# nico-bohlinger/RL-X

Hardware: NVIDIA H100
Metric: env-steps/sec (PPO update incl.) (higher is better)
Workload: dtype f32

## Files before the change

### include/rlx_b200.h

```cpp
#ifndef RLX_B200_H
#define RLX_B200_H

#include <stddef.h>
#include <stdint.h>

#ifdef __cplusplus
extern "C" {
#endif

#define RLX_OK 0
#define RLX_ERR_INVALID_ARG (-1)
#define RLX_ERR_CUDA (-2)
#define RLX_ERR_WORKSPACE (-3)
#define RLX_ERR_UNSUPPORTED (-4)

int rlx_version(void);
const char* rlx_last_error_string(void);
uint64_t rlx_launch_count(void);
void rlx_reset_launch_count(void);
void rlx_add_launch_count(uint64_t n);
#define RLX_NKCLASS 14
int rlx_timing_begin(void);
int rlx_timing_end(double* ms, uint64_t* launches, double* flops, double* bytes);
const char* rlx_kernel_class_name(int cls);
int rlx_set_gemm_engine(int engine);
int rlx_get_gemm_engine(void);
int rlx_set_aux_gemm_engine(int engine);
uint64_t rlx_aux_tc_gemm_count(void);

int rlx_debug_gemm_f32(int engine, int layout, int epilogue, int64_t M, int64_t N, int64_t K, const float* A, int64_t lda,
                       const float* B, int64_t ldb, float* C, int64_t ldc, const float* bias, const float* aux, int64_t ldaux,
                       void* stream);

typedef struct rlx_pcg64 { uint64_t s[6]; } rlx_pcg64;
int rlx_pcg64_seed(uint64_t seed, rlx_pcg64* st);
uint64_t rlx_pcg64_next64(rlx_pcg64* st);
uint32_t rlx_pcg64_next32(rlx_pcg64* st);
int rlx_pcg64_shuffle_i64(rlx_pcg64* st, int64_t* a, int64_t n);
int rlx_pcg64_integers_i64(rlx_pcg64* st, int64_t high, int64_t* out, int64_t n);
int rlx_pcg64_choice_i64(rlx_pcg64* st, int64_t pop_size, int64_t size, int64_t* out);

#define RLX_PPO_NSEG 13
typedef struct rlx_ppo_dims { int32_t obs_dim, act_dim, hidden; } rlx_ppo_dims;
int64_t rlx_ppo_param_count(const rlx_ppo_dims* d);
int rlx_ppo_param_layout(const rlx_ppo_dims* d, int64_t* offsets, int32_t* is_critic);

typedef struct rlx_ppo_forward_args {
  rlx_ppo_dims dims;
  int64_t n;
  const float* params;
  const float* obs;
  const float* noise;
  uint64_t rng_seed, rng_offset;
  const float* act_low;
  const float* act_high;
  int32_t clip_rescale;
  int32_t deterministic;
  float* action;
  float* env_action;
  float* logp;
  float* value;
  void* workspace;
  size_t workspace_bytes;
} rlx_ppo_forward_args;
size_t rlx_ppo_forward_workspace_bytes(const rlx_ppo_dims* d, int64_t n);
int rlx_ppo_forward_f32(const rlx_ppo_forward_args* a, void* stream);

int rlx_critic_forward_f32(const rlx_ppo_dims* d, const float* params, const float* obs, int64_t n, float* value,
                           void* workspace, size_t workspace_bytes, void* stream);

int rlx_rollout_store_f32(const float* reward, const uint8_t* terminated, const uint8_t* truncated, const float* next_obs,
                          int64_t n, int64_t obs_dim, float* rewards_row, float* terminations_row, float* next_obs_dst,
                          int64_t* done_count, void* stream);
int rlx_rollout_store_stats_f32(const float* reward, const uint8_t* terminated, const uint8_t* truncated, const float* next_obs,
                                int64_t n, int64_t obs_dim, float* rewards_row, float* terminations_row, float* next_obs_dst,
                                int64_t* done_count, float* episode_return, float* episode_length, float* done_return_row,
                                float* done_length_row, void* stream);

int rlx_gae_f32(const float* rewards, const float* terminations, const float* values, const float* next_values,
                const float* last_value, int64_t T, int64_t N, double gamma, double gae_lambda, float* advantages,
                float* returns, void* stream);
int rlx_set_gae_tma(int on);

int rlx_gather_minibatch_f32(const int64_t* idx, int64_t count, int64_t obs_dim, int64_t act_dim, const float* states,
                             const float* actions, const float* log_probs, const float* advantages, const float* returns,
                             float* out_states, float* out_actions, float* out_log_probs, float* out_advantages,
                             float* out_returns, int64_t out_states_ld, void* stream);

int rlx_advantage_stats_f32(const float* adv, int64_t count, int64_t mb, float* stats, void* stream);
int rlx_segment_moments_f32(const float* x, const int64_t* offsets, int64_t nseg, const float* gsum, const float* gcount, float* out,
                            void* stream);

typedef struct rlx_ppo_hparams {
  float clip_range;
  float entropy_coef;
  float critic_coef;
  float max_grad_norm;
  float adam_beta1, adam_beta2, adam_eps;
  float ratio_delta_metric;
} rlx_ppo_hparams;

#define RLX_PPO_NMETRIC 8

typedef struct rlx_ppo_minibatch_args {
  rlx_ppo_dims dims;
  int64_t m;
  int64_t m_global;
  const float* states;
  const float* actions;
  const float* log_probs;
  const float* advantages;
  const float* returns;
  const float* adv_stats;
  float* params;
  float* grads;
  float* exp_avg;
  float* exp_avg_sq;
  const float* lr;
  int64_t* step_count;
  rlx_ppo_hparams hp;
  float* metrics;
  void* workspace;
  size_t workspace_bytes;
  int64_t states_ld;
  int32_t states_ones_col;
  int32_t reserved2;
} rlx_ppo_minibatch_args;
size_t rlx_ppo_minibatch_workspace_bytes(const rlx_ppo_dims* d, int64_t m);

int rlx_ppo_minibatch_fwdbwd_f32(const rlx_ppo_minibatch_args* a, void* stream);

int rlx_gradnorm_clip_adam_f32(const rlx_ppo_minibatch_args* a, void* stream);

int rlx_ppo_update_epoch_f32(const rlx_ppo_minibatch_args* first, int64_t count, int64_t mb, void* stream);

#define RLX_COMM_MAX_WORLD 16
#define RLX_COMM_HANDLE_BYTES 64
typedef struct rlx_comm rlx_comm;
int rlx_comm_create(int rank, int world, int64_t nfloats, rlx_comm** out);
int rlx_comm_export_handle(rlx_comm* c, uint8_t* handle);
int rlx_comm_connect(rlx_comm* c, const uint8_t* handles);
float* rlx_comm_send_buffer(rlx_comm* c);
int rlx_comm_stage_f32(rlx_comm* c, const float* src, int64_t n, void* stream);
int rlx_comm_allreduce_sum_f32(rlx_comm* c, float* out, int64_t n, void* stream);
int rlx_comm_set_algorithm(rlx_comm* c, int algo);
int rlx_comm_destroy(rlx_comm* c);

int rlx_ppo_update_epoch_sharded_f32(const rlx_ppo_minibatch_args* first, int64_t num_mb, const int64_t* counts,
                                     const int64_t* global_counts, rlx_comm* comm, void* stream);


int rlx_set_head_engine(int engine);
int rlx_set_autocast_bf16(int on);
int rlx_debug_ppo_head_gemm_f32(int64_t m, int32_t hidden, int32_t act_dim, const float* H2, const float* W3p, const float* W3c, const float* b3p,
                                const float* b3c, const float* logstd, const float* actions, const float* logp_old, const float* adv,
                                const float* ret, const float* adv_stats, float inv_mg, float clip_range, float critic_coef,
                                int32_t ratio_delta_metric, float* dZ2, float* dhead, float* headpart, float* scratch, void* stream);

#define RLX_LSTM_POLICY_NSEG 22
#define RLX_LSTM_CRITIC_NSEG 6
#define RLX_LSTM_OPT_FILM 1
#define RLX_LSTM_OPT_SHARED_ENCODER 2
typedef struct rlx_lstm_dims { int32_t obs_dim, act_dim, hidden, enc_dim, lstm_dim, options ; } rlx_lstm_dims;
int rlx_lstm_param_layout(const rlx_lstm_dims* d, int64_t* policy_offsets , int64_t* critic_offsets );
size_t rlx_lstm_minibatch_workspace_bytes(const rlx_lstm_dims* d, int64_t T, int64_t n_env);

int rlx_set_lstm_persistent(int on);
uint64_t rlx_lstm_persistent_launch_count(void);

typedef struct rlx_lstm_minibatch_args {
  rlx_lstm_dims dims;
  int64_t T, n_env;
  const float* states;
  const float* actions;
  const float* log_probs;
  const float* advantages;
  const float* returns;
  const float* dones;
  const float* init_c;
  const float* init_h;
  const float* adv_stats;
  const float* policy_params;
  const float* critic_params;
  float* policy_grads;
  float* critic_grads;
  float clip_range, entropy_coef, critic_coef, reserved;
  float* metrics;
  void* workspace;
  size_t workspace_bytes;
} rlx_lstm_minibatch_args;
int rlx_lstm_ppo_minibatch_fwdbwd_f32(const rlx_lstm_minibatch_args* a, void* stream);

typedef struct rlx_lstm_step_args {
  rlx_lstm_dims dims;
  int64_t n;
  const float* obs;
  float* c;
  float* h;
  const float* noise;
  const float* policy_params;
  const float* critic_params;
  const float* act_low;
  const float* act_high;
  int32_t clip_rescale;
  int32_t reserved;
  float* action;
  float* env_action;
  float* logp;
  float* value;
  void* workspace;
  size_t workspace_bytes;
} rlx_lstm_step_args;
int rlx_lstm_step_f32(const rlx_lstm_step_args* a, void* stream);
int rlx_lstm_mask_carry_f32(float* c, float* h, const float* done, int64_t n, int64_t lstm_dim, void* stream);
int rlx_lstm_critic_forward_f32(const rlx_lstm_dims* d, const float* critic_params, const float* x, int64_t rows, float* out, void* workspace,
                                size_t workspace_bytes, void* stream);
int rlx_mean_popstd_f32(const float* x, int64_t n, float* out, float* workspace, void* stream);

int rlx_optax_clip_adam_f32(float* params, const float* grads, float* mu, float* nu, int64_t n, const float* lr, int64_t* step_count,
                            float max_norm, float beta1, float beta2, float eps, float* norm_out, float* workspace, void* stream);

int rlx_gather_env_columns_f32(const float* src, const int64_t* env_idx, int64_t T, int64_t N, int64_t n, int64_t width, float* out, void* stream);

#define RLX_FASTSAC_POLICY_NSEG 16
#define RLX_FASTSAC_Q_NSEG 14
typedef struct rlx_fastsac_dims { int32_t obs_dim, act_dim, nr_atoms; } rlx_fastsac_dims;
int rlx_fastsac_param_layout(const rlx_fastsac_dims* d, int64_t* policy_offsets , int64_t* q_offsets );
size_t rlx_fastsac_workspace_bytes(const rlx_fastsac_dims* d, int64_t n);

typedef struct rlx_fastsac_hparams {
  float gamma, tau, v_min, v_max, target_entropy, log_std_min, log_std_max;
  float weight_decay, adam_beta1, adam_beta2, adam_eps, max_grad_norm;
  float clipped_double_q;
} rlx_fastsac_hparams;

typedef struct rlx_fastsac_update_args {
  rlx_fastsac_dims dims;
  int64_t n;
  const float* states;
  const float* next_states;
  const float* actions;
  const float* rewards;
  const float* dones;
  const float* truncations;
  const float* effective_n_steps;
  const float* noise;
  const float* action_scale;
  float* policy_params;  float* policy_grads;  float* policy_m;  float* policy_v;
  float* q_params;       float* q_grads;       float* q_m;       float* q_v;
  float* q_target_params;
  float* log_alpha;      float* alpha_state;
  const float* lr;
  int64_t* steps;
  rlx_fastsac_hparams hp;
  float* metrics;
  void* workspace;
  size_t workspace_bytes;
} rlx_fastsac_update_args;
int rlx_fastsac_critic_update_f32(const rlx_fastsac_update_args* a, void* stream);
int rlx_fastsac_policy_update_f32(const rlx_fastsac_update_args* a, void* stream);
int rlx_fastsac_act_f32(const rlx_fastsac_dims* d, const float* policy_params, const float* obs, const float* noise, const float* action_scale,
                        float log_std_min, float log_std_max, int64_t n, float* action, void* workspace, size_t workspace_bytes, void* stream);
int rlx_fastsac_normalize_f32(const float* x, int64_t n, int64_t obs_dim, float* mean, float* var, float* std, int64_t* count, int32_t update,
                              float eps, float* out, float* workspace, void* stream);

#define RLX_FASTTD3_POLICY_NSEG 8
#define RLX_FASTTD3_Q_NSEG 8
typedef struct rlx_fasttd3_dims { int32_t obs_dim, act_dim, nr_atoms; } rlx_fasttd3_dims;
int rlx_fasttd3_param_layout(const rlx_fasttd3_dims* d, int64_t* policy_offsets , int64_t* q_offsets );
size_t rlx_fasttd3_workspace_bytes(const rlx_fasttd3_dims* d, int64_t n);

typedef struct rlx_fasttd3_hparams {
  float gamma, tau, v_min, v_max, smoothing_epsilon, smoothing_clip_value;
  float weight_decay, adam_beta1, adam_beta2, adam_eps, max_grad_norm;
  float clipped_double_q;
} rlx_fasttd3_hparams;

typedef struct rlx_fasttd3_update_args {
  rlx_fasttd3_dims dims;
  int64_t n;
  const float* states;
  const float* next_states;
  const float* actions;
  const float* rewards;
  const float* dones;
  const float* truncations;
  const float* effective_n_steps;
  const float* smoothing_noise;
  float* policy_params;  float* policy_grads;  float* policy_m;  float* policy_v;
  float* q_params;       float* q_grads;       float* q_m;       float* q_v;
  float* q_target_params;
  const float* lr;
  int64_t* steps;
  rlx_fasttd3_hparams hp;
  float* metrics;
  void* workspace;
  size_t workspace_bytes;
} rlx_fasttd3_update_args;
int rlx_fasttd3_critic_update_f32(const rlx_fasttd3_update_args* a, void* stream);
int rlx_fasttd3_policy_update_f32(const rlx_fasttd3_update_args* a, void* stream);
int rlx_fasttd3_act_f32(const rlx_fasttd3_dims* d, const float* policy_params, const float* obs, const float* noise, const float* noise_scale,
                        const float* act_low, const float* act_high, int32_t clip_rescale, int64_t n, float* action, float* env_action, void* workspace,
                        size_t workspace_bytes, void* stream);

int rlx_replay_sample_gather_f32(const int64_t* idx_t, const int64_t* idx_e, int64_t n, int64_t nr_envs, int64_t obs_dim,
                                 int64_t act_dim, const float* states, const float* next_states, const float* actions,
                                 const float* rewards, const float* terminations, float* out_states, float* out_next_states,
                                 float* out_actions, float* out_rewards, float* out_terminations, void* stream);

int rlx_replay_sample_nstep_f32(const int64_t* idx_t, const int64_t* idx_e, int64_t n, int64_t capacity, int64_t nr_envs, int64_t obs_dim,
                                int64_t act_dim, int32_t n_steps, const float* discounts, int64_t size, int64_t pos, const float* states,
                                const float* next_states, const float* actions, const float* rewards, const float* dones,
                                const float* truncations, float* out_states, float* out_next_states, float* out_actions,
                                float* out_rewards, float* out_dones, float* out_truncations, float* out_effective_n_steps, int64_t* workspace,
                                void* stream);
int rlx_polyak_f32(float* target, const float* online, int64_t n, float tau, void* stream);

typedef struct rlx_sac_dims { int32_t obs_dim, act_dim, hidden; float log_std_min, log_std_max; } rlx_sac_dims;
int64_t rlx_sac_policy_param_count(int32_t obs_dim, int32_t act_dim, int32_t hidden);
int64_t rlx_sac_q_param_count(int32_t obs_dim, int32_t act_dim, int32_t hidden);
size_t rlx_sac_workspace_bytes(int32_t obs_dim, int32_t act_dim, int32_t hidden, int64_t batch);

int rlx_sac_act_f32(const rlx_sac_dims* d, const float* policy_params, const float* obs, const float* eps, int64_t n, const float* act_low,
                    const float* act_high, int32_t deterministic, float* action_tanh, float* env_action, float* logp, void* workspace,
                    size_t workspace_bytes, void* stream);

#define RLX_SAC_NMETRIC 12
typedef struct rlx_sac_update_args {
  rlx_sac_dims dims;
  int64_t batch;
  float* policy;
  float* q;
  float* log_alpha;
  const float* states;
  const float* next_states;
  const float* actions;
  const float* rewards;
  const float* terminations;
  const float* eps_next;
  const float* eps_cur;
  const float* act_low;
  const float* act_high;
  float gamma, tau, target_entropy;
  float adam_beta1, adam_beta2, adam_eps;
  float* g_policy; float* m_policy; float* v_policy;
  float* g_q; float* m_q; float* v_q;
  float* g_log_alpha; float* m_log_alpha; float* v_log_alpha;
  const float* lr;
  int64_t* steps;
  float* metrics;
  void* workspace;
  size_t workspace_bytes;
} rlx_sac_update_args;
int rlx_sac_update_f32(const rlx_sac_update_args* a, void* stream);

#ifdef __cplusplus
}
#endif
#endif
```

### rl_x_b200/_native.py

```python
import ctypes as C
import os

import numpy as np

from . import build as _build

RLX_PPO_NSEG = 13
RLX_PPO_NMETRIC = 8
METRIC_NAMES = ("pg_loss", "critic_loss", "entropy_loss", "approx_kl", "clip_fraction", "policy_grad_norm", "critic_grad_norm", "count")

c_float_p = C.c_void_p


class PpoDims(C.Structure):
    _fields_ = [("obs_dim", C.c_int32), ("act_dim", C.c_int32), ("hidden", C.c_int32)]


class Pcg64(C.Structure):
    _fields_ = [("s", C.c_uint64 * 6)]


class PpoForwardArgs(C.Structure):
    _fields_ = [
        ("dims", PpoDims),
        ("n", C.c_int64),
        ("params", C.c_void_p),
        ("obs", C.c_void_p),
        ("noise", C.c_void_p),
        ("rng_seed", C.c_uint64),
        ("rng_offset", C.c_uint64),
        ("act_low", C.c_void_p),
        ("act_high", C.c_void_p),
        ("clip_rescale", C.c_int32),
        ("deterministic", C.c_int32),
        ("action", C.c_void_p),
        ("env_action", C.c_void_p),
        ("logp", C.c_void_p),
        ("value", C.c_void_p),
        ("workspace", C.c_void_p),
        ("workspace_bytes", C.c_size_t),
    ]


class PpoHparams(C.Structure):
    _fields_ = [
        ("clip_range", C.c_float),
        ("entropy_coef", C.c_float),
        ("critic_coef", C.c_float),
        ("max_grad_norm", C.c_float),
        ("adam_beta1", C.c_float),
        ("adam_beta2", C.c_float),
        ("adam_eps", C.c_float),
        ("ratio_delta_metric", C.c_float),
    ]


class PpoMinibatchArgs(C.Structure):
    _fields_ = [
        ("dims", PpoDims),
        ("m", C.c_int64),
        ("m_global", C.c_int64),
        ("states", C.c_void_p),
        ("actions", C.c_void_p),
        ("log_probs", C.c_void_p),
        ("advantages", C.c_void_p),
        ("returns", C.c_void_p),
        ("adv_stats", C.c_void_p),
        ("params", C.c_void_p),
        ("grads", C.c_void_p),
        ("exp_avg", C.c_void_p),
        ("exp_avg_sq", C.c_void_p),
        ("lr", C.c_void_p),
        ("step_count", C.c_void_p),
        ("hp", PpoHparams),
        ("metrics", C.c_void_p),
        ("workspace", C.c_void_p),
        ("workspace_bytes", C.c_size_t),
        ("states_ld", C.c_int64),
        ("states_ones_col", C.c_int32),
        ("reserved2", C.c_int32),
    ]


class SacDims(C.Structure):
    _fields_ = [("obs_dim", C.c_int32), ("act_dim", C.c_int32), ("hidden", C.c_int32), ("log_std_min", C.c_float), ("log_std_max", C.c_float)]


class SacUpdateArgs(C.Structure):
    _fields_ = [("dims", SacDims), ("batch", C.c_int64)] + [(n, C.c_void_p) for n in (
        "policy", "q", "log_alpha", "states", "next_states", "actions", "rewards", "terminations", "eps_next", "eps_cur", "act_low", "act_high")] + [
        ("gamma", C.c_float), ("tau", C.c_float), ("target_entropy", C.c_float), ("adam_beta1", C.c_float), ("adam_beta2", C.c_float),
        ("adam_eps", C.c_float)] + [(n, C.c_void_p) for n in (
        "g_policy", "m_policy", "v_policy", "g_q", "m_q", "v_q", "g_log_alpha", "m_log_alpha", "v_log_alpha", "lr", "steps", "metrics", "workspace")] + [
        ("workspace_bytes", C.c_size_t)]



class LstmDims(C.Structure):
    _fields_ = [(n, C.c_int32) for n in ("obs_dim", "act_dim", "hidden", "enc_dim", "lstm_dim", "options")]


class LstmMinibatchArgs(C.Structure):
    _fields_ = ([("dims", LstmDims), ("T", C.c_int64), ("n_env", C.c_int64)] +
                [(n, C.c_void_p) for n in ("states", "actions", "log_probs", "advantages", "returns", "dones", "init_c", "init_h", "adv_stats",
                                           "policy_params", "critic_params", "policy_grads", "critic_grads")] +
                [(n, C.c_float) for n in ("clip_range", "entropy_coef", "critic_coef", "reserved")] +
                [("metrics", C.c_void_p), ("workspace", C.c_void_p), ("workspace_bytes", C.c_size_t)])


class LstmStepArgs(C.Structure):
    _fields_ = ([("dims", LstmDims), ("n", C.c_int64)] +
                [(k, C.c_void_p) for k in ("obs", "c", "h", "noise", "policy_params", "critic_params", "act_low", "act_high")] +
                [("clip_rescale", C.c_int32), ("reserved", C.c_int32)] +
                [(k, C.c_void_p) for k in ("action", "env_action", "logp", "value", "workspace")] + [("workspace_bytes", C.c_size_t)])


RLX_LSTM_POLICY_NSEG, RLX_LSTM_CRITIC_NSEG = 22, 6
RLX_LSTM_OPT_FILM, RLX_LSTM_OPT_SHARED_ENCODER = 1, 2
LSTM_POLICY_SEGMENTS = ("We1", "be1", "g1", "n1", "We2", "be2", "g2", "n2", "Wi", "Wh", "bh", "gl", "nl", "Wt1", "bt1", "Wt2", "bt2", "Wm", "bm", "logstd",
                        "Wf", "bf")
LSTM_CRITIC_SEGMENTS = ("Wc1", "bc1", "Wc2", "bc2", "Wc3", "bc3")


RLX_FASTSAC_POLICY_NSEG, RLX_FASTSAC_Q_NSEG = 16, 14


class FastSacDims(C.Structure):
    _fields_ = [(n, C.c_int32) for n in ("obs_dim", "act_dim", "nr_atoms")]


class FastSacHparams(C.Structure):
    _fields_ = [(n, C.c_float) for n in ("gamma", "tau", "v_min", "v_max", "target_entropy", "log_std_min", "log_std_max", "weight_decay",
                                         "adam_beta1", "adam_beta2", "adam_eps", "max_grad_norm", "clipped_double_q")]


class FastSacUpdateArgs(C.Structure):
    _fields_ = ([("dims", FastSacDims), ("n", C.c_int64)] +
                [(k, C.c_void_p) for k in ("states", "next_states", "actions", "rewards", "dones", "truncations", "effective_n_steps", "noise",
                                           "action_scale", "policy_params", "policy_grads", "policy_m", "policy_v", "q_params", "q_grads", "q_m", "q_v",
                                           "q_target_params", "log_alpha", "alpha_state", "lr", "steps")] +
                [("hp", FastSacHparams), ("metrics", C.c_void_p), ("workspace", C.c_void_p), ("workspace_bytes", C.c_size_t)])

RLX_FASTTD3_POLICY_NSEG, RLX_FASTTD3_Q_NSEG = 8, 8


class FastTd3Dims(C.Structure):
    _fields_ = [(n, C.c_int32) for n in ("obs_dim", "act_dim", "nr_atoms")]


class FastTd3Hparams(C.Structure):
    _fields_ = [(n, C.c_float) for n in ("gamma", "tau", "v_min", "v_max", "smoothing_epsilon", "smoothing_clip_value", "weight_decay", "adam_beta1",
                                         "adam_beta2", "adam_eps", "max_grad_norm", "clipped_double_q")]


class FastTd3UpdateArgs(C.Structure):
    _fields_ = ([("dims", FastTd3Dims), ("n", C.c_int64)] +
                [(k, C.c_void_p) for k in ("states", "next_states", "actions", "rewards", "dones", "truncations", "effective_n_steps", "smoothing_noise",
                                           "policy_params", "policy_grads", "policy_m", "policy_v", "q_params", "q_grads", "q_m", "q_v",
                                           "q_target_params", "lr", "steps")] +
                [("hp", FastTd3Hparams), ("metrics", C.c_void_p), ("workspace", C.c_void_p), ("workspace_bytes", C.c_size_t)])

RLX_SAC_NMETRIC = 12
RLX_COMM_MAX_WORLD = 16
RLX_COMM_HANDLE_BYTES = 64
SAC_METRIC_NAMES = ("entropy/alpha", "entropy/entropy", "gradients/policy_grad_norm", "gradients/critic_grad_norm", "gradients/entropy_grad_norm",
                    "loss/q_loss", "loss/policy_loss", "loss/entropy_loss", "q_value/q_value")

_SIGNATURES = {
    "rlx_version": (C.c_int, []),
    "rlx_last_error_string": (C.c_char_p, []),
    "rlx_set_aux_gemm_engine": (C.c_int, [C.c_int]),
    "rlx_aux_tc_gemm_count": (C.c_uint64, []),
    "rlx_launch_count": (C.c_uint64, []),
    "rlx_reset_launch_count": (None, []),
    "rlx_add_launch_count": (None, [C.c_uint64]),
    "rlx_timing_begin": (C.c_int, []),
    "rlx_timing_end": (C.c_int, [C.POINTER(C.c_double), C.POINTER(C.c_uint64), C.POINTER(C.c_double), C.POINTER(C.c_double)]),
    "rlx_kernel_class_name": (C.c_char_p, [C.c_int]),
    "rlx_set_gemm_engine": (C.c_int, [C.c_int]),
    "rlx_set_head_engine": (C.c_int, [C.c_int]),
    "rlx_set_gae_tma": (C.c_int, [C.c_int]),
    "rlx_set_autocast_bf16": (C.c_int, [C.c_int]),
    "rlx_debug_ppo_head_gemm_f32": (C.c_int, [C.c_int64, C.c_int32, C.c_int32] + [C.c_void_p] * 11 + [C.c_float] * 3 + [C.c_int32] + [C.c_void_p] * 5),
    "rlx_get_gemm_engine": (C.c_int, []),
    "rlx_pcg64_seed": (C.c_int, [C.c_uint64, C.POINTER(Pcg64)]),
    "rlx_pcg64_next64": (C.c_uint64, [C.POINTER(Pcg64)]),
    "rlx_pcg64_next32": (C.c_uint32, [C.POINTER(Pcg64)]),
    "rlx_pcg64_shuffle_i64": (C.c_int, [C.POINTER(Pcg64), C.c_void_p, C.c_int64]),
    "rlx_pcg64_integers_i64": (C.c_int, [C.POINTER(Pcg64), C.c_int64, C.c_void_p, C.c_int64]),
    "rlx_pcg64_choice_i64": (C.c_int, [C.POINTER(Pcg64), C.c_int64, C.c_int64, C.c_void_p]),
    "rlx_replay_sample_nstep_f32": (C.c_int, [C.c_void_p, C.c_void_p, C.c_int64, C.c_int64, C.c_int64, C.c_int64, C.c_int64, C.c_int32, C.c_void_p,
                                              C.c_int64, C.c_int64] + [C.c_void_p] * 15),
    "rlx_lstm_param_layout": (C.c_int, [C.POINTER(LstmDims), C.POINTER(C.c_int64), C.POINTER(C.c_int64)]),
    "rlx_lstm_minibatch_workspace_bytes": (C.c_size_t, [C.POINTER(LstmDims), C.c_int64, C.c_int64]),
    "rlx_set_lstm_persistent": (C.c_int, [C.c_int]),
    "rlx_lstm_persistent_launch_count": (C.c_uint64, []),
    "rlx_lstm_ppo_minibatch_fwdbwd_f32": (C.c_int, [C.POINTER(LstmMinibatchArgs), C.c_void_p]),
    "rlx_lstm_step_f32": (C.c_int, [C.POINTER(LstmStepArgs), C.c_void_p]),
    "rlx_lstm_mask_carry_f32": (C.c_int, [C.c_void_p, C.c_void_p, C.c_void_p, C.c_int64, C.c_int64, C.c_void_p]),
    "rlx_lstm_critic_forward_f32": (C.c_int, [C.POINTER(LstmDims), C.c_void_p, C.c_void_p, C.c_int64, C.c_void_p, C.c_void_p, C.c_size_t, C.c_void_p]),
    "rlx_mean_popstd_f32": (C.c_int, [C.c_void_p, C.c_int64, C.c_void_p, C.c_void_p, C.c_void_p]),
    "rlx_optax_clip_adam_f32": (C.c_int, [C.c_void_p] * 4 + [C.c_int64, C.c_void_p, C.c_void_p] + [C.c_float] * 4 + [C.c_void_p] * 3),
    "rlx_gather_env_columns_f32": (C.c_int, [C.c_void_p, C.c_void_p, C.c_int64, C.c_int64, C.c_int64, C.c_int64, C.c_void_p, C.c_void_p]),
    "rlx_fastsac_param_layout": (C.c_int, [C.POINTER(FastSacDims), C.POINTER(C.c_int64), C.POINTER(C.c_int64)]),
    "rlx_fastsac_workspace_bytes": (C.c_size_t, [C.POINTER(FastSacDims), C.c_int64]),
    "rlx_fastsac_critic_update_f32": (C.c_int, [C.POINTER(FastSacUpdateArgs), C.c_void_p]),
    "rlx_fastsac_policy_update_f32": (C.c_int, [C.POINTER(FastSacUpdateArgs), C.c_void_p]),
    "rlx_fastsac_act_f32": (C.c_int, [C.POINTER(FastSacDims), C.c_void_p, C.c_void_p, C.c_void_p, C.c_void_p, C.c_float, C.c_float, C.c_int64, C.c_void_p,
                                      C.c_void_p, C.c_size_t, C.c_void_p]),
    "rlx_fastsac_normalize_f32": (C.c_int, [C.c_void_p, C.c_int64, C.c_int64, C.c_void_p, C.c_void_p, C.c_void_p, C.c_void_p, C.c_int32, C.c_float,
                                            C.c_void_p, C.c_void_p, C.c_void_p]),
    "rlx_fasttd3_param_layout": (C.c_int, [C.POINTER(FastTd3Dims), C.POINTER(C.c_int64), C.POINTER(C.c_int64)]),
    "rlx_fasttd3_workspace_bytes": (C.c_size_t, [C.POINTER(FastTd3Dims), C.c_int64]),
    "rlx_fasttd3_critic_update_f32": (C.c_int, [C.POINTER(FastTd3UpdateArgs), C.c_void_p]),
    "rlx_fasttd3_policy_update_f32": (C.c_int, [C.POINTER(FastTd3UpdateArgs), C.c_void_p]),
    "rlx_fasttd3_act_f32": (C.c_int, [C.POINTER(FastTd3Dims)] + [C.c_void_p] * 6 + [C.c_int32, C.c_int64, C.c_void_p, C.c_void_p, C.c_void_p, C.c_size_t,
                                      C.c_void_p]),
    "rlx_ppo_param_count": (C.c_int64, [C.POINTER(PpoDims)]),
    "rlx_ppo_param_layout": (C.c_int, [C.POINTER(PpoDims), C.POINTER(C.c_int64), C.POINTER(C.c_int32)]),
    "rlx_ppo_forward_workspace_bytes": (C.c_size_t, [C.POINTER(PpoDims), C.c_int64]),
    "rlx_ppo_forward_f32": (C.c_int, [C.POINTER(PpoForwardArgs), C.c_void_p]),
    "rlx_critic_forward_f32": (C.c_int, [C.POINTER(PpoDims), C.c_void_p, C.c_void_p, C.c_int64, C.c_void_p, C.c_void_p, C.c_size_t, C.c_void_p]),
    "rlx_rollout_store_f32": (C.c_int, [C.c_void_p, C.c_void_p, C.c_void_p, C.c_void_p, C.c_int64, C.c_int64, C.c_void_p, C.c_void_p, C.c_void_p, C.c_void_p, C.c_void_p]),
    "rlx_rollout_store_stats_f32": (C.c_int, [C.c_void_p, C.c_void_p, C.c_void_p, C.c_void_p, C.c_int64, C.c_int64, C.c_void_p, C.c_void_p, C.c_void_p, C.c_void_p,
                                              C.c_void_p, C.c_void_p, C.c_void_p, C.c_void_p, C.c_void_p]),
    "rlx_gae_f32": (C.c_int, [C.c_void_p, C.c_void_p, C.c_void_p, C.c_void_p, C.c_void_p, C.c_int64, C.c_int64, C.c_double, C.c_double, C.c_void_p, C.c_void_p, C.c_void_p]),
    "rlx_gather_minibatch_f32": (C.c_int, [C.c_void_p, C.c_int64, C.c_int64, C.c_int64] + [C.c_void_p] * 10 + [C.c_int64, C.c_void_p]),
    "rlx_debug_gemm_f32": (C.c_int, [C.c_int, C.c_int, C.c_int, C.c_int64, C.c_int64, C.c_int64, C.c_void_p, C.c_int64, C.c_void_p, C.c_int64,
                                     C.c_void_p, C.c_int64, C.c_void_p, C.c_void_p, C.c_int64, C.c_void_p]),
    "rlx_advantage_stats_f32": (C.c_int, [C.c_void_p, C.c_int64, C.c_int64, C.c_void_p, C.c_void_p]),
    "rlx_segment_moments_f32": (C.c_int, [C.c_void_p, C.c_void_p, C.c_int64, C.c_void_p, C.c_void_p, C.c_void_p, C.c_void_p]),
    "rlx_ppo_minibatch_workspace_bytes": (C.c_size_t, [C.POINTER(PpoDims), C.c_int64]),
    "rlx_ppo_minibatch_fwdbwd_f32": (C.c_int, [C.POINTER(PpoMinibatchArgs), C.c_void_p]),
    "rlx_gradnorm_clip_adam_f32": (C.c_int, [C.POINTER(PpoMinibatchArgs), C.c_void_p]),
    "rlx_ppo_update_epoch_f32": (C.c_int, [C.POINTER(PpoMinibatchArgs), C.c_int64, C.c_int64, C.c_void_p]),
    "rlx_comm_create": (C.c_int, [C.c_int, C.c_int, C.c_int64, C.POINTER(C.c_void_p)]),
    "rlx_comm_export_handle": (C.c_int, [C.c_void_p, C.c_void_p]),
    "rlx_comm_connect": (C.c_int, [C.c_void_p, C.c_void_p]),
    "rlx_comm_send_buffer": (C.c_void_p, [C.c_void_p]),
    "rlx_comm_stage_f32": (C.c_int, [C.c_void_p, C.c_void_p, C.c_int64, C.c_void_p]),
    "rlx_comm_allreduce_sum_f32": (C.c_int, [C.c_void_p, C.c_void_p, C.c_int64, C.c_void_p]),
    "rlx_comm_set_algorithm": (C.c_int, [C.c_void_p, C.c_int]),
    "rlx_comm_destroy": (C.c_int, [C.c_void_p]),
    "rlx_ppo_update_epoch_sharded_f32": (C.c_int, [C.POINTER(PpoMinibatchArgs), C.c_int64, C.c_void_p, C.c_void_p, C.c_void_p, C.c_void_p]),
    "rlx_replay_sample_gather_f32": (C.c_int, [C.c_void_p, C.c_void_p, C.c_int64, C.c_int64, C.c_int64, C.c_int64] + [C.c_void_p] * 10 + [C.c_void_p]),
    "rlx_polyak_f32": (C.c_int, [C.c_void_p, C.c_void_p, C.c_int64, C.c_float, C.c_void_p]),
    "rlx_sac_policy_param_count": (C.c_int64, [C.c_int32, C.c_int32, C.c_int32]),
    "rlx_sac_q_param_count": (C.c_int64, [C.c_int32, C.c_int32, C.c_int32]),
    "rlx_sac_workspace_bytes": (C.c_size_t, [C.c_int32, C.c_int32, C.c_int32, C.c_int64]),
    "rlx_sac_act_f32": (C.c_int, [C.POINTER(SacDims), C.c_void_p, C.c_void_p, C.c_void_p, C.c_int64, C.c_void_p, C.c_void_p, C.c_int32, C.c_void_p,
                                  C.c_void_p, C.c_void_p, C.c_void_p, C.c_size_t, C.c_void_p]),
    "rlx_sac_update_f32": (C.c_int, [C.POINTER(SacUpdateArgs), C.c_void_p]),
}

_lib = None


def library_path():
    return _build.LIB_PATH


def load(build_if_missing=True):
    global _lib
    if _lib is not None:
        return _lib
    path = _build.LIB_PATH
    if not os.path.exists(path) or (build_if_missing and not _build.is_fresh()):
        if not build_if_missing:
            raise RuntimeError(f"rl_x_b200: native library missing: {path} (run `python -m rl_x_b200.build`)")
        try:
            _build.build()
        except Exception as e:
            if not os.path.exists(path):
                raise RuntimeError(f"rl_x_b200: cannot build native library: {e}") from e
    try:
        lib = C.CDLL(path)
    except OSError as e:
        raise RuntimeError(f"rl_x_b200: cannot load native library {path}: {e}") from e
    missing = []
    for name, (res, args) in _SIGNATURES.items():
        try:
            fn = getattr(lib, name)
        except AttributeError:
            missing.append(name)
            continue
        fn.restype = res
        fn.argtypes = args
    if missing:
        raise RuntimeError(f"rl_x_b200: native library lacks symbols: {missing}")
    if os.environ.get("RLX_AUX_GEMM_ENGINE", "") in ("0", "1"):
        lib.rlx_set_aux_gemm_engine(int(os.environ["RLX_AUX_GEMM_ENGINE"]))
    if os.environ.get("RLX_LSTM_PERSISTENT", "") in ("0", "1"):
        lib.rlx_set_lstm_persistent(int(os.environ["RLX_LSTM_PERSISTENT"]))
    _lib = lib
    return lib


def exported_symbols():
    return list(_SIGNATURES)


def last_error():
    return load().rlx_last_error_string().decode("utf-8", "replace")


def check(rc, what=""):
    if rc != 0:
        raise RuntimeError(f"rl_x_b200 native call failed ({what}, code {rc}): {last_error()}")


RLX_NKCLASS = 14


def timing_begin():
    check(load().rlx_timing_begin(), "rlx_timing_begin")


def timing_end():
    lib = load()
    ms, fl, by = (C.c_double * RLX_NKCLASS)(), (C.c_double * RLX_NKCLASS)(), (C.c_double * RLX_NKCLASS)()
    n = (C.c_uint64 * RLX_NKCLASS)()
    check(lib.rlx_timing_end(ms, n, fl, by), "rlx_timing_end")
    return {lib.rlx_kernel_class_name(i).decode(): dict(ms=ms[i], launches=int(n[i]), flops=fl[i], bytes=by[i]) for i in range(RLX_NKCLASS)}


def ptr(t):
    if t is None:
        return None
    if isinstance(t, np.ndarray):
        return t.ctypes.data
    return t.data_ptr()


def stream_ptr(device=None):
    import torch

    if not torch.cuda.is_available():
        return None
    return torch.cuda.current_stream(device).cuda_stream


class Pcg64Generator:

    def __init__(self, seed):
        self._lib = load()
        self.state = Pcg64()
        check(self._lib.rlx_pcg64_seed(C.c_uint64(int(seed)), C.byref(self.state)), "pcg64_seed")

    def shuffle(self, a):
        if not (isinstance(a, np.ndarray) and a.dtype == np.int64 and a.ndim == 1 and a.flags.c_contiguous):
            raise TypeError("shuffle expects a contiguous 1-D int64 numpy array")
        check(self._lib.rlx_pcg64_shuffle_i64(C.byref(self.state), a.ctypes.data, a.shape[0]), "pcg64_shuffle")

    def integers(self, high, size):
        out = np.empty(int(size), dtype=np.int64)
        check(self._lib.rlx_pcg64_integers_i64(C.byref(self.state), int(high), out.ctypes.data, out.shape[0]), "pcg64_integers")
        return out

    def choice(self, a, size, replace=False):
        if replace or not isinstance(a, (int, np.integer)):
            raise NotImplementedError("only choice(int, size, replace=False) is mirrored")
        out = np.empty(int(size), dtype=np.int64)
        check(self._lib.rlx_pcg64_choice_i64(C.byref(self.state), int(a), out.shape[0], out.ctypes.data), "pcg64_choice")
        return out

    def next_uint64(self):
        return int(self._lib.rlx_pcg64_next64(C.byref(self.state)))

    def next_uint32(self):
        return int(self._lib.rlx_pcg64_next32(C.byref(self.state)))


SEGMENT_NAMES = ("W1p", "W1c", "b1p", "b1c", "W2p", "W2c", "b2p", "b2c", "W3p", "W3c", "b3p", "b3c", "logstd")


def ppo_layout(obs_dim, act_dim, hidden):
    lib = load()
    d = PpoDims(obs_dim, act_dim, hidden)
    off = (C.c_int64 * (RLX_PPO_NSEG + 1))()
    crit = (C.c_int32 * RLX_PPO_NSEG)()
    check(lib.rlx_ppo_param_layout(C.byref(d), off, crit), "ppo_param_layout")
    return list(off), list(crit)


def segment_shapes(obs_dim, act_dim, hidden):
    H, O, A = hidden, obs_dim, act_dim
    return {"W1p": (H, O), "W1c": (H, O), "b1p": (H,), "b1c": (H,), "W2p": (H, H), "W2c": (H, H), "b2p": (H,), "b2c": (H,),
            "W3p": (A, H), "W3c": (1, H), "b3p": (A,), "b3c": (1,), "logstd": (1, A)}


POLICY_KEYS = {"policy_mean.0.weight": "W1p", "policy_mean.0.bias": "b1p", "policy_mean.2.weight": "W2p", "policy_mean.2.bias": "b2p",
               "policy_mean.4.weight": "W3p", "policy_mean.4.bias": "b3p", "policy_logstd": "logstd"}
CRITIC_KEYS = {"critic.0.weight": "W1c", "critic.0.bias": "b1c", "critic.2.weight": "W2c", "critic.2.bias": "b2c",
               "critic.4.weight": "W3c", "critic.4.bias": "b3c"}
```

### rl_x_b200/algorithms/ppo/b200/kernels.py

```python
import ctypes as C

import numpy as np
import torch

from rl_x_b200 import _native as nt


def _f32(t, name):
    if t is None:
        return None
    if not (t.is_cuda and t.dtype == torch.float32 and t.is_contiguous()):
        raise TypeError(f"{name}: expected a contiguous float32 CUDA tensor, got {t.dtype} on {t.device} (contiguous={t.is_contiguous()})")
    return t.data_ptr()


def _bool_u8(t, name):
    if t is None:
        return None
    if not (t.is_cuda and t.dtype in (torch.bool, torch.uint8) and t.is_contiguous()):
        raise TypeError(f"{name}: expected a contiguous bool/uint8 CUDA tensor")
    return t.data_ptr()


def _stream():
    return torch.cuda.current_stream().cuda_stream


class PpoKernels:

    def __init__(self, obs_dim, act_dim, hidden):
        self.lib = nt.load()
        self.dims = nt.PpoDims(int(obs_dim), int(act_dim), int(hidden))
        self.obs_dim, self.act_dim, self.hidden = int(obs_dim), int(act_dim), int(hidden)
        n = self.lib.rlx_ppo_param_count(C.byref(self.dims))
        if n <= 0:
            raise RuntimeError(f"rl_x_b200: unsupported network shape obs={obs_dim} act={act_dim} hidden={hidden}: {nt.last_error()}")
        self.param_count = int(n)
        self.offsets, self.is_critic = nt.ppo_layout(obs_dim, act_dim, hidden)

    def forward_workspace(self, n, device):
        nbytes = self.lib.rlx_ppo_forward_workspace_bytes(C.byref(self.dims), int(n))
        return torch.empty(max(int(nbytes), 16), dtype=torch.uint8, device=device)

    def minibatch_workspace(self, m, device):
        nbytes = self.lib.rlx_ppo_minibatch_workspace_bytes(C.byref(self.dims), int(m))
        return torch.empty(max(int(nbytes), 16), dtype=torch.uint8, device=device)

    def forward(self, params, obs, workspace, **kw):
        nt.check(self.lib.rlx_ppo_forward_f32(C.byref(self.forward_args(params, obs, workspace, **kw)), _stream()), "rlx_ppo_forward_f32")

    def forward_prepared(self, a):
        nt.check(self.lib.rlx_ppo_forward_f32(C.byref(a), _stream()), "rlx_ppo_forward_f32")

    def forward_args(self, params, obs, workspace, *, noise=None, rng_seed=0, rng_offset=0, act_low=None, act_high=None,
                     clip_rescale=True, deterministic=False, action=None, env_action=None, logp=None, value=None):
        a = nt.PpoForwardArgs()
        a.dims = self.dims
        a.n = obs.shape[0]
        a.params = _f32(params, "params")
        a.obs = _f32(obs, "obs")
        a.noise = _f32(noise, "noise")
        a.rng_seed, a.rng_offset = int(rng_seed), int(rng_offset)
        a.act_low, a.act_high = _f32(act_low, "act_low"), _f32(act_high, "act_high")
        a.clip_rescale, a.deterministic = int(bool(clip_rescale)), int(bool(deterministic))
        a.action, a.env_action = _f32(action, "action"), _f32(env_action, "env_action")
        a.logp, a.value = _f32(logp, "logp"), _f32(value, "value")
        a.workspace, a.workspace_bytes = workspace.data_ptr(), workspace.numel()
        return a

    def critic_forward(self, params, obs, value, workspace):
        nt.check(self.lib.rlx_critic_forward_f32(C.byref(self.dims), _f32(params, "params"), _f32(obs, "obs"), obs.shape[0],
                                                 _f32(value, "value"), workspace.data_ptr(), workspace.numel(), _stream()),
                 "rlx_critic_forward_f32")

    def rollout_store(self, reward, terminated, truncated, next_obs, rewards_row, terminations_row, next_obs_dst, done_count, episode_stats=None):
        n = reward.shape[0] if reward is not None else next_obs.shape[0]
        es = [_f32(t, "episode_stats") for t in episode_stats] if episode_stats is not None else [None] * 4
        nt.check(self.lib.rlx_rollout_store_stats_f32(_f32(reward, "reward"), _bool_u8(terminated, "terminated"), _bool_u8(truncated, "truncated"),
                                                      _f32(next_obs, "next_obs"), n, self.obs_dim, _f32(rewards_row, "rewards_row"),
                                                      _f32(terminations_row, "terminations_row"), _f32(next_obs_dst, "next_obs_dst"),
                                                      done_count.data_ptr() if done_count is not None else None, *es, _stream()),
                 "rlx_rollout_store_stats_f32")

    def gae(self, rewards, terminations, values, gamma, gae_lambda, advantages, returns, next_values=None, last_value=None):
        T, N = rewards.shape
        nt.check(self.lib.rlx_gae_f32(_f32(rewards, "rewards"), _f32(terminations, "terminations"), _f32(values, "values"),
                                      _f32(next_values, "next_values"), _f32(last_value, "last_value"), T, N, float(gamma),
                                      float(gae_lambda), _f32(advantages, "advantages"), _f32(returns, "returns"), _stream()),
                 "rlx_gae_f32")

    def gather(self, idx, states, actions, log_probs, advantages, returns, out_states, out_actions, out_log_probs,
               out_advantages, out_returns, count=None, out_states_ld=0):
        if not (idx.is_cuda and idx.dtype == torch.int64 and idx.is_contiguous()):
            raise TypeError("idx: expected a contiguous int64 CUDA tensor")
        count = idx.shape[0] if count is None else int(count)
        nt.check(self.lib.rlx_gather_minibatch_f32(idx.data_ptr(), count, self.obs_dim, self.act_dim, _f32(states, "states"),
                                                   _f32(actions, "actions"), _f32(log_probs, "log_probs"), _f32(advantages, "advantages"),
                                                   _f32(returns, "returns"), _f32(out_states, "out_states"), _f32(out_actions, "out_actions"),
                                                   _f32(out_log_probs, "out_log_probs"), _f32(out_advantages, "out_advantages"),
                                                   _f32(out_returns, "out_returns"), int(out_states_ld), _stream()), "rlx_gather_minibatch_f32")

    def advantage_stats(self, adv, count, mb, stats):
        nt.check(self.lib.rlx_advantage_stats_f32(_f32(adv, "adv"), int(count), int(mb), _f32(stats, "stats"), _stream()),
                 "rlx_advantage_stats_f32")

    def segment_moments(self, x, offsets, gsum, gcount, out):
        if not (offsets.is_cuda and offsets.dtype == torch.int64 and offsets.is_contiguous()):
            raise TypeError("offsets: expected a contiguous int64 CUDA tensor")
        nt.check(self.lib.rlx_segment_moments_f32(_f32(x, "x"), offsets.data_ptr(), offsets.numel() - 1, _f32(gsum, "gsum"), _f32(gcount, "gcount"),
                                                  _f32(out, "out"), _stream()), "rlx_segment_moments_f32")

    def minibatch_args(self, *, m, m_global, states, actions, log_probs, advantages, returns, adv_stats, params, grads, exp_avg,
                       exp_avg_sq, lr, step_count, hp, metrics, workspace, states_ld=0, states_ones_col=False):
        a = nt.PpoMinibatchArgs()
        a.dims = self.dims
        a.m, a.m_global = int(m), int(m_global)
        a.states, a.actions = _f32(states, "states"), _f32(actions, "actions")
        a.log_probs, a.advantages, a.returns = _f32(log_probs, "log_probs"), _f32(advantages, "advantages"), _f32(returns, "returns")
        a.adv_stats = _f32(adv_stats, "adv_stats")
        a.params, a.grads = _f32(params, "params"), _f32(grads, "grads")
        a.exp_avg, a.exp_avg_sq = _f32(exp_avg, "exp_avg"), _f32(exp_avg_sq, "exp_avg_sq")
        a.lr = _f32(lr, "lr")
        a.step_count = step_count.data_ptr() if step_count is not None else None
        a.hp = hp
        a.metrics = _f32(metrics, "metrics")
        a.workspace, a.workspace_bytes = workspace.data_ptr(), workspace.numel()
        a.states_ld, a.states_ones_col = int(states_ld), int(bool(states_ones_col))
        return a

    def debug_gemm(self, engine, layout, epilogue, A, B, C, M, N, K, bias=None, aux=None):
        nt.check(self.lib.rlx_debug_gemm_f32(int(engine), int(layout), int(epilogue), M, N, K, _f32(A, "A"), A.stride(0), _f32(B, "B"), B.stride(0),
                                             _f32(C, "C"), C.stride(0), _f32(bias, "bias"), _f32(aux, "aux"), aux.stride(0) if aux is not None else 0,
                                             _stream()), "rlx_debug_gemm_f32")

    def states_pitch(self):
        return (self.obs_dim + 1 + 3) // 4 * 4

    def fwdbwd(self, args):
        nt.check(self.lib.rlx_ppo_minibatch_fwdbwd_f32(C.byref(args), _stream()), "rlx_ppo_minibatch_fwdbwd_f32")

    def clip_adam(self, args):
        nt.check(self.lib.rlx_gradnorm_clip_adam_f32(C.byref(args), _stream()), "rlx_gradnorm_clip_adam_f32")

    def update_epoch(self, first_args, count, mb):
        nt.check(self.lib.rlx_ppo_update_epoch_f32(C.byref(first_args), int(count), int(mb), _stream()), "rlx_ppo_update_epoch_f32")

    def update_epoch_sharded(self, first_args, counts, global_counts, comm):
        assert counts.dtype == np.int64 and global_counts.dtype == np.int64 and len(counts) == len(global_counts)
        nt.check(self.lib.rlx_ppo_update_epoch_sharded_f32(C.byref(first_args), len(counts), counts.ctypes.data, global_counts.ctypes.data,
                                                           comm.handle, _stream()), "rlx_ppo_update_epoch_sharded_f32")


def make_hparams(clip_range, entropy_coef, critic_coef, max_grad_norm, beta1=0.9, beta2=0.999, eps=1e-8, ratio_delta_metric=False):
    code = 2.0 if ratio_delta_metric == "median" else (1.0 if ratio_delta_metric else 0.0)
    return nt.PpoHparams(float(clip_range), float(entropy_coef), float(critic_coef), float(max_grad_norm), float(beta1), float(beta2),
                         float(eps), code)


class PeerComm:

    def __init__(self, dist, nfloats, device):
        self.lib = nt.load()
        self.rank, self.world = dist.get_rank(), dist.get_world_size()
        if self.world > nt.RLX_COMM_MAX_WORLD:
            raise RuntimeError(f"PeerComm supports up to {nt.RLX_COMM_MAX_WORLD} ranks")
        self.nfloats = int(nfloats)
        self.handle = C.c_void_p()
        with torch.cuda.device(device):
            nt.check(self.lib.rlx_comm_create(self.rank, self.world, self.nfloats, C.byref(self.handle)), "rlx_comm_create")
            mine = np.zeros(nt.RLX_COMM_HANDLE_BYTES, dtype=np.uint8)
            nt.check(self.lib.rlx_comm_export_handle(self.handle, mine.ctypes.data), "rlx_comm_export_handle")
            gathered = [torch.zeros(nt.RLX_COMM_HANDLE_BYTES, dtype=torch.uint8, device=device) for _ in range(self.world)]
            dist.all_gather(gathered, torch.from_numpy(mine).to(device))
            handles = np.ascontiguousarray(torch.stack(gathered).cpu().numpy())
            rc = self.lib.rlx_comm_connect(self.handle, handles.ctypes.data)
            ok = torch.tensor([1 if rc == 0 else 0], device=device)
            dist.all_reduce(ok, op=dist.ReduceOp.MIN)
            if int(ok.item()) == 0:
                err = self.lib.rlx_last_error_string().decode() if rc != 0 else "a peer rank could not map this rank's buffer"
                self.close()
                raise RuntimeError("PeerComm: " + err)

    def stage(self, src, n=None):
        n = src.numel() if n is None else int(n)
        nt.check(self.lib.rlx_comm_stage_f32(self.handle, _f32(src, "src"), n, _stream()), "rlx_comm_stage_f32")

    def allreduce_sum(self, out, n=None):
        n = out.numel() if n is None else int(n)
        nt.check(self.lib.rlx_comm_allreduce_sum_f32(self.handle, _f32(out, "out"), n, _stream()), "rlx_comm_allreduce_sum_f32")

    def set_algorithm(self, algo):
        nt.check(self.lib.rlx_comm_set_algorithm(self.handle, int(algo)), "rlx_comm_set_algorithm")

    def close(self):
        if self.handle:
            self.lib.rlx_comm_destroy(self.handle)
            self.handle = C.c_void_p()

    def __del__(self):
        try:
            self.close()
        except Exception:
            pass
```

### rl_x_b200/csrc/gemm_dispatch.cuh

```cuda
#pragma once
#include "gemm_simt.cuh"

namespace rlx {

int tc_supported(const rlx_ppo_dims& d);
int tc_gemm(const GemmP& g, bool a_kmaj, bool b_kmaj, int epi, int batch, int kclass, long long a_rows, long long b_rows, cudaStream_t stream);
int tc_gemm_t(const GemmP& g, bool a_kmaj, bool b_kmaj, int epi, int batch, int kclass, long long a_rows, long long b_rows, int m_main, float* extra_row,
              long long extra_batch_off, long long extra_split_off, cudaStream_t stream);
enum { TC_NONE = 0, TC_BIAS_TANH = 1, TC_DTANH = 2, TC_BIAS_RELU = 3, TC_DRELU = 4, TC_BIAS = 5 };

template <int EPI>
constexpr int tc_epi_of() {
  return EPI == EPI_BIAS_TANH ? TC_BIAS_TANH : EPI == EPI_DTANH ? TC_DTANH : EPI == EPI_BIAS_RELU ? TC_BIAS_RELU : EPI == EPI_DRELU ? TC_DRELU
       : EPI == EPI_BIAS ? TC_BIAS : TC_NONE;
}

template <bool A_KMAJ, bool B_KMAJ, int EPI>
static int run_gemm(bool tc, const GemmP& g, int batch, cudaStream_t st, int kclass, long long a_rows, long long b_rows) {
  if (tc && g.rowsum == nullptr && g.K >= 32) {
    const int rc = tc_gemm(g, A_KMAJ, B_KMAJ, tc_epi_of<EPI>(), batch, kclass, a_rows, b_rows, st);
    if (rc != RLX_ERR_UNSUPPORTED) return rc;
  }
  return launch_sgemm<A_KMAJ, B_KMAJ, EPI>(g, batch, st, kclass);
}

}
```

### rl_x_b200/csrc/gemm_simt.cuh

```cuda
#pragma once
#include "common.cuh"

namespace rlx {

enum Epi { EPI_NONE = 0, EPI_BIAS = 1, EPI_BIAS_TANH = 2, EPI_DTANH = 3, EPI_BIAS_RELU = 4, EPI_DRELU = 5 };

struct GemmP {
  const float* A;
  const float* B;
  float* C;
  const float* bias;
  const float* aux;
  float* rowsum;
  int M, N, K;
  int lda, ldb, ldc, ldaux;
  long long sA, sB, sC, sBias, sAux, sRowsum;
  int splits;
  int kchunk;
  long long sSplitC, sSplitRowsum;
  int bf16;
};

constexpr int GBM = 128, GBN = 128, GBK = 8, GPAD = 4;

template <bool KMAJ, bool VEC>
__device__ __forceinline__ void gemm_load_tile(const float* __restrict__ X, int ld, int row0, int nrows, int k0, int kend,
                                               int tid, float (&r)[4]) {
  if (KMAJ) {
    const int row = row0 + (tid >> 1), k = k0 + (tid & 1) * 4;
    if (row < nrows) {
      const float* p = X + (long long)row * ld + k;
      if (VEC && k + 3 < kend) {
        const float4 v = *reinterpret_cast<const float4*>(p);
        r[0] = v.x; r[1] = v.y; r[2] = v.z; r[3] = v.w;
      } else {
#pragma unroll
        for (int j = 0; j < 4; ++j) r[j] = (k + j < kend) ? p[j] : 0.f;
      }
    } else {
      r[0] = r[1] = r[2] = r[3] = 0.f;
    }
  } else {
    const int k = k0 + (tid >> 5), row = row0 + (tid & 31) * 4;
    if (k < kend) {
      const float* p = X + (long long)k * ld + row;
      if (VEC && row + 3 < nrows) {
        const float4 v = *reinterpret_cast<const float4*>(p);
        r[0] = v.x; r[1] = v.y; r[2] = v.z; r[3] = v.w;
      } else {
#pragma unroll
        for (int j = 0; j < 4; ++j) r[j] = (row + j < nrows) ? p[j] : 0.f;
      }
    } else {
      r[0] = r[1] = r[2] = r[3] = 0.f;
    }
  }
}

template <bool KMAJ>
__device__ __forceinline__ void gemm_store_tile(float (*S)[GBM + GPAD], int tid, const float (&r)[4]) {
  if (KMAJ) {
    const int row = tid >> 1, k = (tid & 1) * 4;
#pragma unroll
    for (int j = 0; j < 4; ++j) S[k + j][row] = r[j];
  } else {
    const int k = tid >> 5, row = (tid & 31) * 4;
    *reinterpret_cast<float4*>(&S[k][row]) = make_float4(r[0], r[1], r[2], r[3]);
  }
}

template <bool A_KMAJ, bool B_KMAJ, int EPI, bool VEC>
__global__ void __launch_bounds__(256, 2) sgemm_kernel(const GemmP p) {
  __shared__ __align__(16) float As[2][GBK][GBM + GPAD];
  __shared__ __align__(16) float Bs[2][GBK][GBN + GPAD];

  const int tid = threadIdx.x, tx = tid & 15, ty = tid >> 4;
  const int batch = blockIdx.z / p.splits, split = blockIdx.z % p.splits;
  const int m0 = blockIdx.y * GBM, n0 = blockIdx.x * GBN;
  const int kbeg = split * p.kchunk;
  const int kend = min(p.K, kbeg + p.kchunk);

  const float* __restrict__ A = p.A + batch * p.sA;
  const float* __restrict__ B = p.B + batch * p.sB;

  float acc[8][8];
#pragma unroll
  for (int i = 0; i < 8; ++i)
#pragma unroll
    for (int j = 0; j < 8; ++j) acc[i][j] = 0.f;
  float rs[8];
#pragma unroll
  for (int i = 0; i < 8; ++i) rs[i] = 0.f;
  const bool do_rowsum = (p.rowsum != nullptr) && blockIdx.x == 0 && tx == 0;

  float ra[4], rb[4];
  const int nk = (kend - kbeg + GBK - 1) / GBK;
  if (nk > 0) {
    gemm_load_tile<A_KMAJ, VEC>(A, p.lda, m0, p.M, kbeg, kend, tid, ra);
    gemm_load_tile<B_KMAJ, VEC>(B, p.ldb, n0, p.N, kbeg, kend, tid, rb);
    gemm_store_tile<A_KMAJ>(As[0], tid, ra);
    gemm_store_tile<B_KMAJ>(Bs[0], tid, rb);
  }
  __syncthreads();

  for (int kt = 0; kt < nk; ++kt) {
    const int buf = kt & 1;
    if (kt + 1 < nk) {
      gemm_load_tile<A_KMAJ, VEC>(A, p.lda, m0, p.M, kbeg + (kt + 1) * GBK, kend, tid, ra);
      gemm_load_tile<B_KMAJ, VEC>(B, p.ldb, n0, p.N, kbeg + (kt + 1) * GBK, kend, tid, rb);
    }
#pragma unroll
    for (int k = 0; k < GBK; ++k) {
      const float4 a0 = *reinterpret_cast<const float4*>(&As[buf][k][ty * 4]);
      const float4 a1 = *reinterpret_cast<const float4*>(&As[buf][k][ty * 4 + 64]);
      const float4 b0 = *reinterpret_cast<const float4*>(&Bs[buf][k][tx * 4]);
      const float4 b1 = *reinterpret_cast<const float4*>(&Bs[buf][k][tx * 4 + 64]);
      const float a[8] = {a0.x, a0.y, a0.z, a0.w, a1.x, a1.y, a1.z, a1.w};
      const float b[8] = {b0.x, b0.y, b0.z, b0.w, b1.x, b1.y, b1.z, b1.w};
#pragma unroll
      for (int i = 0; i < 8; ++i)
#pragma unroll
        for (int j = 0; j < 8; ++j) acc[i][j] = fmaf(a[i], b[j], acc[i][j]);
      if (do_rowsum) {
#pragma unroll
        for (int i = 0; i < 8; ++i) rs[i] += a[i];
      }
    }
    if (kt + 1 < nk) {
      gemm_store_tile<A_KMAJ>(As[buf ^ 1], tid, ra);
      gemm_store_tile<B_KMAJ>(Bs[buf ^ 1], tid, rb);
    }
    __syncthreads();
  }

  float* __restrict__ C = p.C + batch * p.sC + split * p.sSplitC;
  const float* __restrict__ bias = (EPI == EPI_BIAS || EPI == EPI_BIAS_TANH || EPI == EPI_BIAS_RELU) ? p.bias + batch * p.sBias : nullptr;
  const float* __restrict__ aux = (EPI == EPI_DTANH || EPI == EPI_DRELU) ? p.aux + batch * p.sAux : nullptr;
#pragma unroll
  for (int i = 0; i < 8; ++i) {
    const int m = m0 + ((i < 4) ? (ty * 4 + i) : (64 + ty * 4 + (i - 4)));
    if (m >= p.M) continue;
#pragma unroll
    for (int jh = 0; jh < 2; ++jh) {
      const int nb = n0 + jh * 64 + tx * 4;
      float v[4];
#pragma unroll
      for (int j = 0; j < 4; ++j) {
        const int n = nb + j;
        float x = acc[i][jh * 4 + j];
        if (n < p.N) {
          if (EPI == EPI_BIAS) x = bf16r_if(x + bias[n], p.bf16);
          if (EPI == EPI_BIAS_TANH) x = bf16r_if(tanhf(bf16r_if(x + bias[n], p.bf16)), p.bf16);
          if (EPI == EPI_BIAS_RELU) x = fmaxf(x + bias[n], 0.f);
          if (EPI == EPI_DTANH) {
            const float h = aux[(long long)m * p.ldaux + n];
            x = bf16r_if(bf16r_if(x, p.bf16) * (1.f - h * h), p.bf16);
          }
          if (EPI == EPI_DRELU) {
            const float h = aux[(long long)m * p.ldaux + n];
            x = (h > 0.f) ? x : 0.f;
          }
        }
        v[j] = x;
      }
      float* cp = C + (long long)m * p.ldc + nb;
      if (VEC && nb + 3 < p.N) {
        *reinterpret_cast<float4*>(cp) = make_float4(v[0], v[1], v[2], v[3]);
      } else {
#pragma unroll
        for (int j = 0; j < 4; ++j)
          if (nb + j < p.N) cp[j] = v[j];
      }
    }
  }
  if (do_rowsum) {
    float* rsout = p.rowsum + batch * p.sRowsum + split * p.sSplitRowsum;
#pragma unroll
    for (int i = 0; i < 8; ++i) {
      const int m = m0 + ((i < 4) ? (ty * 4 + i) : (64 + ty * 4 + (i - 4)));
      if (m < p.M) rsout[m] = rs[i];
    }
  }
}

inline bool gemm_vec_ok(const GemmP& p) {
  auto al = [](const void* q) { return (reinterpret_cast<uintptr_t>(q) & 15) == 0; };
  bool ok = al(p.A) && al(p.B) && al(p.C) && (p.lda % 4 == 0) && (p.ldb % 4 == 0) && (p.ldc % 4 == 0);
  ok = ok && (p.sA % 4 == 0) && (p.sB % 4 == 0) && (p.sC % 4 == 0) && (p.sSplitC % 4 == 0) && (p.kchunk % 4 == 0);
  return ok;
}

template <bool A_KMAJ, bool B_KMAJ, int EPI>
int launch_sgemm(const GemmP& p, int batch, cudaStream_t stream, int kclass = KC_OTHER) {
  if (p.M <= 0 || p.N <= 0) return RLX_OK;
  dim3 grid((unsigned)ceil_div(p.N, GBN), (unsigned)ceil_div(p.M, GBM), (unsigned)(batch * p.splits));
  const double flops = 2.0 * p.M * p.N * (double)p.K * batch;
  const double bytes = 4.0 * batch * ((double)p.M * p.K + (double)p.N * p.K + (double)p.M * p.N * p.splits);
  if (gemm_vec_ok(p)) {
    RLX_LAUNCH_C(kclass, flops, bytes, (sgemm_kernel<A_KMAJ, B_KMAJ, EPI, true>), grid, 256, 0, stream, p);
  } else {
    RLX_LAUNCH_C(kclass, flops, bytes, (sgemm_kernel<A_KMAJ, B_KMAJ, EPI, false>), grid, 256, 0, stream, p);
  }
  return RLX_OK;
}

}
```

### rl_x_b200/csrc/gemm_tc.cu

```cuda
#include "gemm_dispatch.cuh"
#include "gemm_tc_common.cuh"

namespace rlx {
namespace tc {

struct Cfg {
  static constexpr int A_BYTES = BM * BK * 4;
  static constexpr int B_BYTES = BN * BK * 4;
  static constexpr int RAW_BYTES = A_BYTES + B_BYTES;
  static constexpr int OP_BYTES = 2 * B_BYTES;
  static constexpr int RAW_STAGES = 3, OP_STAGES = 4;
  static constexpr int SMEM_BYTES = RAW_STAGES * RAW_BYTES + OP_STAGES * OP_BYTES + 1024  + 1024 ;
  static constexpr int PRODUCER_REGS = 56, CONSUMER_REGS = 224;
};
static_assert(Cfg::SMEM_BYTES <= 227 * 1024, "shared memory of one H100 block");
static_assert(Cfg::PRODUCER_REGS * 128 + Cfg::CONSUMER_REGS * 256 <= 65536, "register file of one SM");

template <bool KMAJ, bool BF16, int ROWS>
__device__ __forceinline__ void convert_tile(const uint8_t* raw, uint8_t* hi, uint8_t* lo, int t) {
  constexpr uint32_t HI = 0xFFFFE000u;
  if (KMAJ) {
#pragma unroll 4
    for (int i = t; i < ROWS * 8; i += 128) {
      const uint4 v = reinterpret_cast<const uint4*>(raw)[i];
      const uint4 h = make_uint4(v.x & HI, v.y & HI, v.z & HI, v.w & HI);
      reinterpret_cast<uint4*>(hi)[i] = h;
      if (!BF16)
        reinterpret_cast<float4*>(lo)[i] = make_float4(__uint_as_float(v.x) - __uint_as_float(h.x), __uint_as_float(v.y) - __uint_as_float(h.y),
                                                       __uint_as_float(v.z) - __uint_as_float(h.z), __uint_as_float(v.w) - __uint_as_float(h.w));
    }
  } else {
#pragma unroll 2
    for (int i = t; i < ROWS * 8; i += 128) {
      const int mn = i % ROWS, kc = i / ROWS;
      const uint8_t* box = raw + (mn >> 5) * (BK * 128);
      const int c = (mn & 31) >> 2, e = mn & 3;
      uint32_t v[4];
#pragma unroll
      for (int q = 0; q < 4; ++q) {
        const int k = kc * 4 + q;
        v[q] = *reinterpret_cast<const uint32_t*>(box + k * 128 + ((c ^ (k & 7)) << 4) + e * 4);
      }
      const int off = mn * 128 + ((kc ^ (mn & 7)) << 4);
      const uint4 h = make_uint4(v[0] & HI, v[1] & HI, v[2] & HI, v[3] & HI);
      *reinterpret_cast<uint4*>(hi + off) = h;
      if (!BF16)
        *reinterpret_cast<float4*>(lo + off) = make_float4(__uint_as_float(v[0]) - __uint_as_float(h.x), __uint_as_float(v[1]) - __uint_as_float(h.y),
                                                           __uint_as_float(v[2]) - __uint_as_float(h.z), __uint_as_float(v[3]) - __uint_as_float(h.w));
    }
  }
}

template <bool KMAJ, bool BF16>
__device__ __forceinline__ void load_a_frags(const uint8_t* raw, int r0, int lane, int half, uint32_t (&hi)[2][4], uint32_t (&lo)[2][4]) {
  constexpr uint32_t HI = 0xFFFFE000u;
  const int t4 = lane & 3;
  uint32_t v[2][4];
  if (KMAJ) {
#pragma unroll
    for (int r = 0; r < 2; ++r) {
      const uint8_t* row = raw + (r0 + 8 * r) * 128 + t4 * 4;
#pragma unroll
      for (int jj = 0; jj < 4; ++jj) v[r][jj] = *reinterpret_cast<const uint32_t*>(row + (((4 * half + jj) ^ (r0 & 7)) << 4));
    }
  } else {
    const int s = (lane >> 4) & 1;
#pragma unroll
    for (int r = 0; r < 2; ++r) {
      const int m = r0 + 8 * r;
      const uint8_t* box = raw + (m >> 5) * (BK * 128) + (m & 3) * 4;
      const int mc = (m & 31) >> 2;
#pragma unroll
      for (int jj = 0; jj < 4; jj += 2) {
        const int j = 4 * half + jj;
        const int k0 = t4 + 4 * (j + s), k1 = t4 + 4 * (j + 1 - s);
        const uint32_t x0 = *reinterpret_cast<const uint32_t*>(box + k0 * 128 + ((mc ^ (k0 & 7)) << 4));
        const uint32_t x1 = *reinterpret_cast<const uint32_t*>(box + k1 * 128 + ((mc ^ (k1 & 7)) << 4));
        v[r][jj] = s ? x1 : x0;
        v[r][jj + 1] = s ? x0 : x1;
      }
    }
  }
#pragma unroll
  for (int r = 0; r < 2; ++r)
#pragma unroll
    for (int jj = 0; jj < 4; ++jj) {
      const uint32_t h = v[r][jj] & HI;
      hi[jj >> 1][2 * (jj & 1) + r] = h;
      if (!BF16) lo[jj >> 1][2 * (jj & 1) + r] = __float_as_uint(__uint_as_float(v[r][jj]) - __uint_as_float(h));
    }
}


template <bool FULL>
__device__ __forceinline__ void load_cols(float (&v)[32], const float* src, int lim, int c0) {
#pragma unroll
  for (int i = 2 * c0; i < 2 * c0 + 16; ++i) {
    const int o = 8 * (i >> 1) + (i & 1);
    v[i] = (FULL || o <= lim) ? src[o] : 0.f;
  }
}

template <int EPI, bool BF16>
__device__ __forceinline__ float epilogue_op(float x, float e) {
  if (EPI == TC_EPI_DTANH || EPI == TC_EPI_DRELU)
    x = (EPI == TC_EPI_DTANH) ? bf16r_if(bf16r_if(x, BF16) * (1.f - e * e), BF16) : ((e > 0.f) ? x : 0.f);
  if (EPI == TC_EPI_BIAS_TANH || EPI == TC_EPI_BIAS_RELU || EPI == TC_EPI_BIAS) {
    const float z = (EPI == TC_EPI_BIAS_RELU) ? x + e : bf16r_if(x + e, BF16);
    x = (EPI == TC_EPI_BIAS_TANH) ? bf16r_if(tanh_fast(z), BF16) : ((EPI == TC_EPI_BIAS_RELU) ? fmaxf(z, 0.f) : z);
  }
  return x;
}

template <int EPI, bool BF16, bool TRANS, bool FULL, class LoadAux>
__device__ __forceinline__ void store_tile(const float (&acc)[64], const float (&cor)[64], float (&e)[2][32], const TcParams& p, float* cbase,
                                           float* ebase, int m, int ct, LoadAux load_aux) {
  auto x = [&](int j) { return BF16 ? acc[j] : acc[j] + cor[j]; };
  constexpr bool HAS_AUX = (EPI == TC_EPI_DTANH || EPI == TC_EPI_DRELU);
  if (!TRANS) {
#pragma unroll
    for (int h = 0; h < 2; ++h) {
      const int mh = m + 8 * h;
      float* row = cbase + (long long)mh * p.ldc + ct;
      const bool row_ok = FULL || mh < p.M;
#pragma unroll
      for (int c = 0; c < 16; ++c) {
        if (HAS_AUX && c % 8 == 0 && 2 * h + c / 8 < 3) load_aux(2 * h + c / 8 + 1);
        const int j = 4 * c + 2 * h;
        const float x0 = epilogue_op<EPI, BF16>(x(j), e[HAS_AUX ? h : 0][2 * c]);
        const float x1 = epilogue_op<EPI, BF16>(x(j + 1), e[HAS_AUX ? h : 0][2 * c + 1]);
        const int n = ct + 8 * c;
        if (FULL || (row_ok && n + 1 < p.N)) *reinterpret_cast<float2*>(row + 8 * c) = make_float2(x0, x1);
        else if (row_ok && n < p.N) row[8 * c] = x0;
      }
    }
  } else {
    float* col = cbase + (long long)ct * p.ldc + m;
    const int ldc = (int)p.ldc;
#pragma unroll
    for (int c = 0; c < 16; ++c)
#pragma unroll
      for (int q = 0; q < 2; ++q) {
        const int off = (8 * c + q) * ldc;
        const int n = ct + 8 * c + q;
#pragma unroll
        for (int h = 0; h < 2; ++h) {
          const float v = x(4 * c + 2 * h + q);
          const int mh = m + 8 * h;
          if (FULL || (n < p.N && mh < p.m_main)) col[off + 8 * h] = v;
          else if (n < p.N && mh == p.m_main && mh < p.M && ebase != nullptr) ebase[n] = v;
        }
      }
  }
}

template <bool A_KMAJ, bool B_KMAJ, int EPI, bool BF16, bool TRANS>
__global__ void __launch_bounds__(NUM_THREADS, 1) tc_gemm_kernel(const __grid_constant__ CUtensorMap tmap_a,
                                                                 const __grid_constant__ CUtensorMap tmap_b, const TcParams p) {
  constexpr int RAW_STAGES = Cfg::RAW_STAGES, OP_STAGES = Cfg::OP_STAGES;
  extern __shared__ uint8_t smem_raw[];
  uint8_t* smem = smem_raw + ((1024u - (smem_u32(smem_raw) & 1023u)) & 1023u);
  uint8_t* ops = smem + RAW_STAGES * Cfg::RAW_BYTES;
  uint64_t* raw_full = reinterpret_cast<uint64_t*>(ops + OP_STAGES * Cfg::OP_BYTES);
  uint64_t* raw_empty = raw_full + RAW_STAGES;
  uint64_t* op_full = raw_empty + RAW_STAGES;
  uint64_t* op_empty = op_full + OP_STAGES;

  const int warp = threadIdx.x >> 5, lane = threadIdx.x & 31;
  if (threadIdx.x == 0) {
    prefetch_tmap(&tmap_a);
    prefetch_tmap(&tmap_b);
    for (int s = 0; s < RAW_STAGES; ++s) {
      mbar_init(&raw_full[s], 1);
      mbar_init(&raw_empty[s], 1 + 8);
    }
    for (int s = 0; s < OP_STAGES; ++s) {
      mbar_init(&op_full[s], 1);
      mbar_init(&op_empty[s], 8);
    }
    fence_barrier_init();
  }
  __syncthreads();

  const int tiles_per_z = p.tiles_m * p.tiles_n;
  const int num_tiles = tiles_per_z * p.batch * p.splits;

  auto tile_coords = [&](int tile, int& zb, int& zs, int& m0, int& n0, int& kbeg, int& nkb) {
    const int z = tile / tiles_per_z, r = tile % tiles_per_z;
    zb = z / p.splits;
    zs = z % p.splits;
    m0 = (r / p.tiles_n) * BM;
    n0 = (r % p.tiles_n) * BN;
    kbeg = zs * p.kchunk;
    const int kend = min(p.K, kbeg + p.kchunk);
    nkb = (kend - kbeg + BK - 1) / BK;
  };

  if (warp < 4) {
    setmaxnreg_dec<Cfg::PRODUCER_REGS>();
    const int t = threadIdx.x;
    int ld_tile = blockIdx.x, ld_kb = 0, ld_count = 0;
    auto load_next = [&]() {
      while (ld_tile < num_tiles) {
        int zb, zs, m0, n0, kbeg, nkb;
        tile_coords(ld_tile, zb, zs, m0, n0, kbeg, nkb);
        if (ld_kb >= nkb) {
          ld_tile += gridDim.x;
          ld_kb = 0;
          continue;
        }
        const int slot = ld_count % RAW_STAGES;
        mbar_wait(&raw_empty[slot], ((ld_count / RAW_STAGES) & 1) ^ 1);
        uint8_t* sa = smem + slot * Cfg::RAW_BYTES;
        uint8_t* sb = sa + Cfg::A_BYTES;
        uint64_t* bar = &raw_full[slot];
        const int k0 = kbeg + ld_kb * BK;
        mbar_arrive_expect_tx(bar, Cfg::RAW_BYTES);
        if (A_KMAJ) {
          tma_load_2d(&tmap_a, bar, sa, p.a_k_off * zb + k0, p.a_mn_off * zb + m0);
        } else {
#pragma unroll
          for (int j = 0; j < BM / 32; ++j) tma_load_2d(&tmap_a, bar, sa + j * (BK * 128), p.a_mn_off * zb + m0 + 32 * j, p.a_k_off * zb + k0);
        }
        if (B_KMAJ) {
          tma_load_2d(&tmap_b, bar, sb, p.b_k_off * zb + k0, p.b_mn_off * zb + n0);
        } else {
#pragma unroll
          for (int j = 0; j < BN / 32; ++j) tma_load_2d(&tmap_b, bar, sb + j * (BK * 128), p.b_mn_off * zb + n0 + 32 * j, p.b_k_off * zb + k0);
        }
        ++ld_kb;
        ++ld_count;
        return;
      }
    };
    if (t == 0)
      for (int i = 0; i < RAW_STAGES; ++i) load_next();
    int rs = 0, os = 0;
    uint32_t rph = 0, oph = 0;
    bool refill = false;
    for (int tile = blockIdx.x; tile < num_tiles; tile += gridDim.x) {
      int zb, zs, m0, n0, kbeg, nkb;
      tile_coords(tile, zb, zs, m0, n0, kbeg, nkb);
      for (int kb = 0; kb < nkb; ++kb) {
        mbar_wait(&raw_full[rs], rph);
        mbar_wait(&op_empty[os], oph ^ 1);
        uint8_t* op = ops + os * Cfg::OP_BYTES;
        convert_tile<B_KMAJ, BF16, BN>(smem + rs * Cfg::RAW_BYTES + Cfg::A_BYTES, op, op + Cfg::B_BYTES, t);
        fence_proxy_async();
        named_bar_sync(1, 128);
        if (t == 0) {
          mbar_arrive(&op_full[os]);
          mbar_arrive(&raw_empty[rs]);
          if (refill) load_next();
          refill = true;
        }
        if (++rs == RAW_STAGES) { rs = 0; rph ^= 1; }
        if (++os == OP_STAGES) { os = 0; oph ^= 1; }
      }
    }
  } else {
    setmaxnreg_inc<Cfg::CONSUMER_REGS>();
    const int cw = (warp >> 2) - 1;
    const int r0 = cw * 64 + (warp & 3) * 16 + (lane >> 2);
    float acc[64], cor[64];
    uint32_t ah[2][2][4], al[2][2][4];
    int rs = 0, os = 0;
    uint32_t rph = 0, oph = 0;
    for (int tile = blockIdx.x; tile < num_tiles; tile += gridDim.x) {
      int zb, zs, m0, n0, kbeg, nkb;
      tile_coords(tile, zb, zs, m0, n0, kbeg, nkb);
      for (int kb = 0; kb < nkb; ++kb) {
        mbar_wait(&raw_full[rs], rph);
        mbar_wait(&op_full[os], oph);
        const uint8_t* raw = smem + rs * Cfg::RAW_BYTES;
        const uint32_t op = smem_u32(ops + os * Cfg::OP_BYTES);
        const uint64_t db = make_smem_desc(op), db_lo = make_smem_desc(op + Cfg::B_BYTES);
#pragma unroll
        for (int h = 0; h < 2; ++h) {
          load_a_frags<A_KMAJ, BF16>(raw, r0, lane, h, ah[h], al[h]);
          if (h == 1) {
            __syncwarp();
            if (lane == 0) mbar_arrive(&raw_empty[rs]);
          }
          fence_frags(ah[h]);
          if (!BF16) fence_frags(al[h]);
          wgmma_fence();
#pragma unroll
          for (int q = 0; q < 2; ++q) {
            const int kk = 2 * h + q;
            const uint64_t ko = (uint64_t)((kk * WG_K * 4) >> 4);
            const uint32_t accum = (kb | kk) != 0 ? 1u : 0u;
            if (!BF16) {
              wgmma_tf32_m64n128k8(cor, al[h][q], db + ko, accum);
              wgmma_tf32_m64n128k8(cor, ah[h][q], db_lo + ko, 1u);
            }
            wgmma_tf32_m64n128k8(acc, ah[h][q], db + ko, accum);
          }
          wgmma_commit();
          wgmma_wait_1();
          if (h == 0 && kb > 0 && lane == 0) mbar_arrive(&op_empty[os == 0 ? OP_STAGES - 1 : os - 1]);
        }
        if (++rs == RAW_STAGES) { rs = 0; rph ^= 1; }
        if (++os == OP_STAGES) { os = 0; oph ^= 1; }
      }

      constexpr bool HAS_AUX = (EPI == TC_EPI_DTANH || EPI == TC_EPI_DRELU);
      constexpr bool HAS_BIAS = (EPI == TC_EPI_BIAS_TANH || EPI == TC_EPI_BIAS_RELU || EPI == TC_EPI_BIAS);
      const int m = m0 + r0, ct = n0 + 2 * (lane & 3);
      const bool full = m0 + BM <= (TRANS ? p.m_main : p.M) && n0 + BN <= p.N;
      const int clim = p.N - 1 - ct;
      const float* abase = HAS_AUX ? p.aux + p.aux_batch_off * zb + ct : nullptr;
      float e[2][32];
      auto load_aux = [&](int q) {
        const float* arow = abase + (long long)min(m + 8 * (q >> 1), p.M - 1) * p.ldaux;
        if (full) load_cols<true>(e[q >> 1], arow, clim, 8 * (q & 1));
        else load_cols<false>(e[q >> 1], arow, clim, 8 * (q & 1));
      };
      if (HAS_BIAS) {
        const float* b = p.bias + p.bias_batch_off * zb + ct;
#pragma unroll
        for (int c0 = 0; c0 < 16; c0 += 8) {
          if (full) load_cols<true>(e[0], b, clim, c0);
          else load_cols<false>(e[0], b, clim, c0);
        }
      }
      if (HAS_AUX) load_aux(0);
      if (nkb > 0) {
        wgmma_wait_all();
        if (lane == 0) mbar_arrive(&op_empty[os == 0 ? OP_STAGES - 1 : os - 1]);
      }
      fence_acc(acc);
      if (!BF16) fence_acc(cor);
      float* cbase = p.C + p.c_batch_off * zb + p.c_split_off * zs;
      float* ebase = (TRANS && p.extra_row != nullptr) ? p.extra_row + p.extra_batch_off * zb + p.extra_split_off * zs : nullptr;
      if (full) store_tile<EPI, BF16, TRANS, true>(acc, cor, e, p, cbase, ebase, m, ct, load_aux);
      else store_tile<EPI, BF16, TRANS, false>(acc, cor, e, p, cbase, ebase, m, ct, load_aux);
    }
  }
}

template <bool A_KMAJ, bool B_KMAJ, int EPI, bool BF16 = false, bool TRANS = false>
static int launch_cfg(const TcOperand& A, const TcOperand& B, TcParams p, int kclass, cudaStream_t stream) {
  CUtensorMap ta, tb;
  int rc = make_tmap(&ta, A.base, A.rows, A.cols, A.ld, 32, A_KMAJ ? BM : BK);
  if (rc) return rc;
  rc = make_tmap(&tb, B.base, B.rows, B.cols, B.ld, 32, B_KMAJ ? BN : BK);
  if (rc) return rc;
  p.tiles_m = (int)ceil_div(p.M, BM);
  p.tiles_n = (int)ceil_div(p.N, BN);
  const long long tiles = (long long)p.tiles_m * p.tiles_n * p.batch * p.splits;
  if (tiles <= 0) return RLX_OK;
  static_assert(!TRANS || EPI == TC_EPI_NONE, "the transposed store has no epilogue function");
  auto kern = tc_gemm_kernel<A_KMAJ, B_KMAJ, EPI, BF16, TRANS>;
  static bool attr_done = false;
  if (!attr_done) {
    RLX_CHECK_CUDA(cudaFuncSetAttribute(kern, cudaFuncAttributeMaxDynamicSharedMemorySize, Cfg::SMEM_BYTES));
    attr_done = true;
  }
  const unsigned grid = (unsigned)std::min<long long>(tiles, sm_count());
  const double flops = 2.0 * p.M * p.N * (double)p.K * p.batch;
  const double bytes = 4.0 * p.batch * ((double)p.M * p.K + (double)p.N * p.K + (double)p.M * p.N * p.splits);
  RLX_LAUNCH_C(kclass, flops, bytes, kern, grid, NUM_THREADS, Cfg::SMEM_BYTES, stream, ta, tb, p);
  return RLX_OK;
}

}

using namespace tc;

int tc_supported(const rlx_ppo_dims& d) {
  return (d.hidden % 128 == 0) && d.hidden >= 128 && d.hidden <= 1024 && (d.obs_dim % 4 == 0) && d.obs_dim >= 32;
}

static bool aligned16(const void* p) { return (reinterpret_cast<uintptr_t>(p) & 15) == 0; }

static int tc_gemm_impl(const GemmP& g, bool a_kmaj, bool b_kmaj, int epi, int batch, int kclass, long long a_rows, long long b_rows, bool trans,
                        int m_main, float* extra_row, long long extra_batch_off, long long extra_split_off, cudaStream_t stream) {
  if (g.M <= 0 || g.N <= 0) return RLX_OK;
  if (!aligned16(g.A) || !aligned16(g.B) || !aligned16(g.C) || g.lda % 4 || g.ldb % 4 || g.ldc % 4) return RLX_ERR_UNSUPPORTED;
  if (g.splits > 1 && g.kchunk % BK) return RLX_ERR_UNSUPPORTED;
  if (!trans && (((batch > 1 ? g.sC : 0) | (g.splits > 1 ? g.sSplitC : 0)) & 1)) return RLX_ERR_UNSUPPORTED;
  if (batch > 1) {
    auto expressible = [](long long off, int ld) { return off == 0 || off % ld == 0 || off < ld; };
    if (!expressible(g.sA, g.lda) || !expressible(g.sB, g.ldb)) {
      if (g.sA % 4 || g.sB % 4 || g.sC % 4 || g.sAux % 4) return RLX_ERR_UNSUPPORTED;
      for (int b = 0; b < batch; ++b) {
        GemmP gb = g;
        gb.A = g.A + b * g.sA; gb.B = g.B + b * g.sB; gb.C = g.C + b * g.sC;
        if (g.bias) gb.bias = g.bias + b * g.sBias;
        if (g.aux) gb.aux = g.aux + b * g.sAux;
        gb.sA = gb.sB = gb.sC = gb.sBias = gb.sAux = 0;
        const long long ar = a_rows, br = b_kmaj ? (long long)g.N : (long long)g.K;
        const int rc = tc_gemm_impl(gb, a_kmaj, b_kmaj, epi, 1, kclass, ar, br, trans, m_main, extra_row ? extra_row + b * extra_batch_off : nullptr, 0,
                                    extra_split_off, stream);
        if (rc) return rc;
      }
      return RLX_OK;
    }
  }
  TcParams p{};
  p.M = g.M; p.N = g.N; p.K = g.K;
  p.batch = batch; p.splits = g.splits;
  p.kchunk = (g.splits > 1) ? g.kchunk : (int)(ceil_div(g.K, BK) * BK);
  auto split_off = [](long long off, int ld, bool kmaj, int& mn_off, int& k_off) {
    const long long r = off / ld, c = off % ld;
    if (kmaj) { mn_off = (int)r; k_off = (int)c; } else { k_off = (int)r; mn_off = (int)c; }
  };
  split_off(g.sA, g.lda, a_kmaj, p.a_mn_off, p.a_k_off);
  split_off(g.sB, g.ldb, b_kmaj, p.b_mn_off, p.b_k_off);
  p.C = g.C; p.ldc = g.ldc; p.c_batch_off = g.sC; p.c_split_off = g.sSplitC;
  p.m_main = (trans && m_main > 0) ? m_main : g.M;
  p.extra_row = extra_row; p.extra_batch_off = extra_batch_off; p.extra_split_off = extra_split_off;
  p.bias = g.bias; p.bias_batch_off = g.sBias;
  p.aux = g.aux; p.ldaux = g.ldaux; p.aux_batch_off = g.sAux;
  p.single = g.bf16 ? 1 : 0;
  p.bf16 = g.bf16;
  TcOperand A{g.A, (a_kmaj ? (long long)p.a_mn_off : (long long)p.a_k_off) * (batch - 1) + a_rows,
              a_kmaj ? (long long)(p.a_k_off * (batch - 1) + g.K) : (long long)(p.a_mn_off * (batch - 1) + g.M), g.lda};
  TcOperand B{g.B, (b_kmaj ? (long long)p.b_mn_off : (long long)p.b_k_off) * (batch - 1) + b_rows,
              b_kmaj ? (long long)(p.b_k_off * (batch - 1) + g.K) : (long long)(p.b_mn_off * (batch - 1) + g.N), g.ldb};
  if (trans) {
    if (!a_kmaj && !b_kmaj && epi == TC_EPI_NONE)
      return p.bf16 ? launch_cfg<false, false, TC_EPI_NONE, true, true>(A, B, p, kclass, stream)
                    : launch_cfg<false, false, TC_EPI_NONE, false, true>(A, B, p, kclass, stream);
    return RLX_ERR_UNSUPPORTED;
  }
  if (p.bf16 && a_kmaj && b_kmaj && epi == TC_EPI_BIAS_TANH) return launch_cfg<true, true, TC_EPI_BIAS_TANH, true>(A, B, p, kclass, stream);
  if (p.bf16 && a_kmaj && !b_kmaj && epi == TC_EPI_DTANH) return launch_cfg<true, false, TC_EPI_DTANH, true>(A, B, p, kclass, stream);
  if (p.bf16 && !a_kmaj && !b_kmaj && epi == TC_EPI_NONE) return launch_cfg<false, false, TC_EPI_NONE, true>(A, B, p, kclass, stream);
  if (p.bf16) return RLX_ERR_UNSUPPORTED;
  if (a_kmaj && b_kmaj && epi == TC_EPI_BIAS_TANH) return launch_cfg<true, true, TC_EPI_BIAS_TANH>(A, B, p, kclass, stream);
  if (a_kmaj && b_kmaj && epi == TC_EPI_NONE) return launch_cfg<true, true, TC_EPI_NONE>(A, B, p, kclass, stream);
  if (a_kmaj && b_kmaj && epi == TC_EPI_BIAS_RELU) return launch_cfg<true, true, TC_EPI_BIAS_RELU>(A, B, p, kclass, stream);
  if (a_kmaj && b_kmaj && epi == TC_EPI_BIAS) return launch_cfg<true, true, TC_EPI_BIAS>(A, B, p, kclass, stream);
  if (a_kmaj && !b_kmaj && epi == TC_EPI_DRELU) return launch_cfg<true, false, TC_EPI_DRELU>(A, B, p, kclass, stream);
  if (a_kmaj && !b_kmaj && epi == TC_EPI_DTANH) return launch_cfg<true, false, TC_EPI_DTANH>(A, B, p, kclass, stream);
  if (a_kmaj && !b_kmaj && epi == TC_EPI_NONE) return launch_cfg<true, false, TC_EPI_NONE>(A, B, p, kclass, stream);
  if (!a_kmaj && !b_kmaj && epi == TC_EPI_NONE) return launch_cfg<false, false, TC_EPI_NONE>(A, B, p, kclass, stream);
  return RLX_ERR_UNSUPPORTED;
}

int tc_gemm(const GemmP& g, bool a_kmaj, bool b_kmaj, int epi, int batch, int kclass, long long a_rows, long long b_rows, cudaStream_t stream) {
  return tc_gemm_impl(g, a_kmaj, b_kmaj, epi, batch, kclass, a_rows, b_rows, false, 0, nullptr, 0, 0, stream);
}

int tc_gemm_t(const GemmP& g, bool a_kmaj, bool b_kmaj, int epi, int batch, int kclass, long long a_rows, long long b_rows, int m_main, float* extra_row,
              long long extra_batch_off, long long extra_split_off, cudaStream_t stream) {
  return tc_gemm_impl(g, a_kmaj, b_kmaj, epi, batch, kclass, a_rows, b_rows, true, m_main, extra_row, extra_batch_off, extra_split_off, stream);
}

}
```

### rl_x_b200/csrc/ppo.cu

```cuda
#include "common.cuh"
#include "gemm_simt.cuh"
#include "gemm_dispatch.cuh"
#include "ppo_head.cuh"
#include "ppo_head_gemm.cuh"
#include "ppo_head_mma.cuh"
#include "ppo_optim.cuh"

namespace rlx {

static bool use_tc(const rlx_ppo_dims& d) { return g_gemm_engine == 1 && tc_supported(d); }
}
int comm_allreduce_ppo(rlx_comm* c, float* out, int64_t n, const rlx_ppo_dims& d, float* norm_partials, long long* step_count, void* stream, int* nblk_out);
namespace rlx {

struct Splits {
  int splits, kchunk;
};
static Splits choose_splits(long long rows, int out_m, int out_n, int batch, bool tc) {
  if (tc) {
    const long long tiles = ceil_div(out_m, 128) * ceil_div(out_n, 128) * batch;
    const long long smin = std::max<long long>(1, ceil_div(rows, 1024)), smax = std::max<long long>(smin, std::min<long long>(smin + 64, rows / 64));
    const long long sms = sm_count();
    long long best = smin;
    double best_fill = -1.0;
    for (long long s = smin; s <= smax; ++s) {
      const long long t = tiles * s;
      const double fill = (double)t / (double)(ceil_div(t, sms) * sms);
      if (fill > best_fill + 0.02) { best_fill = fill; best = s; }
    }
    long long kchunk = std::max<long long>(32, ceil_div(ceil_div(rows, best), 32) * 32);
    return Splits{(int)ceil_div(rows, kchunk), (int)kchunk};
  }
  const long long tiles = ceil_div(out_m, GBM) * ceil_div(out_n, GBN) * batch;
  const long long target = (long long)sm_count() * 2;
  long long s = std::max<long long>(1, target / std::max<long long>(tiles, 1));
  s = std::min<long long>(s, std::max<long long>(1, rows / 256));
  long long kchunk = std::max<long long>(8, ceil_div(ceil_div(rows, s), 8) * 8);
  return Splits{(int)ceil_div(rows, kchunk), (int)kchunk};
}

__global__ void __launch_bounds__(256) round_bf16_kernel(const float* __restrict__ src, float* __restrict__ dst, long long n, long long keep_lo,
                                                         long long keep_hi) {
  const long long stride = (long long)gridDim.x * blockDim.x;
  for (long long i = (long long)blockIdx.x * blockDim.x + threadIdx.x; i < n; i += stride) {
    const float x = src[i];
    dst[i] = (i >= keep_lo && i < keep_hi) ? x : bf16r(x);
  }
}
static int launch_round_bf16(const float* src, float* dst, long long n, long long keep_lo, long long keep_hi, cudaStream_t st) {
  if (n <= 0) return RLX_OK;
  const unsigned grid = (unsigned)std::min<long long>(ceil_div(n, 256), (long long)sm_count() * 8);
  RLX_LAUNCH_C(KC_OTHER, 0, 8.0 * n, round_bf16_kernel, grid, 256, 0, st, src, dst, n, keep_lo, keep_hi);
  return RLX_OK;
}
static int round_inputs_bf16(const PpoLayout& L, const float*& params, const float*& X, long long n_x, float* pr, float* xr, cudaStream_t st) {
  int rc = launch_round_bf16(params, pr, L.total(), L.off[LOGSTD], L.off[LOGSTD + 1], st);
  if (rc) return rc;
  rc = launch_round_bf16(X, xr, n_x, 0, 0, st);
  if (rc) return rc;
  params = pr;
  X = xr;
  return RLX_OK;
}

struct FwdPlan {
  size_t off_H1, off_H2, off_P, off_X, total;
};
static FwdPlan plan_forward(const rlx_ppo_dims& d, long long n) {
  FwdPlan P;
  size_t o = 0;
  const size_t act_bytes = align_up((size_t)n * 2 * d.hidden * sizeof(float), 256);
  P.off_H1 = o; o += act_bytes;
  P.off_H2 = o; o += act_bytes;
  P.off_P = o; o += align_up((size_t)make_layout(d).total() * sizeof(float), 256);
  P.off_X = o; o += align_up((size_t)n * d.obs_dim * sizeof(float), 256);
  P.total = o;
  return P;
}

constexpr int kHeadWgradRows = 64;

struct TrainPlan {
  size_t off_H1, off_H2, off_dZ2, off_dZ1, off_dhead, off_headpart, off_part1, off_rs1, off_part2, off_part3, off_norm, off_barrier, off_P, off_X, off_ratio, total;
  int max_s1, max_s2, max_s3;
  int head_blocks, wgrad_chunks, norm_blocks, head_npart;
};
static int head_grid(long long m) { return (int)std::min<long long>(ceil_div(m, 16), (long long)sm_count() * 2); }

static TrainPlan plan_train(const rlx_ppo_dims& d, long long m) {
  TrainPlan P;
  const long long H = d.hidden, O = d.obs_dim, A = d.act_dim;
  P.max_s1 = std::max(choose_splits(m, (int)(2 * H), (int)O, 1, false).splits, choose_splits(m, (int)O + 1, (int)(2 * H), 1, true).splits);
  P.max_s2 = std::max(choose_splits(m, (int)H, (int)H, 2, false).splits, choose_splits(m, (int)H, (int)H, 2, true).splits);
  P.head_blocks = head_grid(m);
  P.head_npart = (int)(2 * A + 5 + 2 * H);
  P.wgrad_chunks = (int)ceil_div(m, kHeadWgradRows);
  P.norm_blocks = (int)std::max<long long>(std::max(64, sm_count()), ceil_div(make_layout(d).total(), 256) + ceil_div(2 * H + 2 * A + 1 + (A + 1) * H, 8) + 8);
  size_t o = 0;
  auto take = [&](size_t& off, size_t nfloats) {
    off = o;
    o += align_up(nfloats * sizeof(float), 256);
  };
  take(P.off_H1, (size_t)m * 2 * H);
  take(P.off_H2, (size_t)m * 2 * H);
  take(P.off_dZ2, (size_t)m * 2 * H);
  take(P.off_dZ1, (size_t)m * 2 * H);
  take(P.off_dhead, (size_t)m * (ceil_div(A + 1, 4) * 4));
  take(P.off_headpart, (size_t)P.head_blocks * P.head_npart);
  take(P.off_part1, (size_t)P.max_s1 * 2 * H * O);
  take(P.off_rs1, (size_t)P.max_s1 * 2 * H);
  take(P.off_part2, (size_t)P.max_s2 * 2 * H * H);
  const size_t dh_ld_plan = (size_t)(ceil_div(A + 1, 4) * 4);
  P.max_s3 = choose_splits(m, (int)dh_ld_plan, (int)H, 2, true).splits;
  take(P.off_part3, std::max<size_t>((size_t)P.wgrad_chunks * (A + 1) * H, (size_t)P.max_s3 * 2 * dh_ld_plan * H));
  take(P.off_norm, (size_t)P.norm_blocks * 2);
  take(P.off_barrier, 64);
  take(P.off_P, (size_t)make_layout(d).total());
  take(P.off_X, (size_t)m * (size_t)(ceil_div(O + 1, 4) * 4));
  take(P.off_ratio, (size_t)m);
  P.total = o;
  return P;
}

template <typename T>
static T* ws_ptr(void* ws, size_t off) {
  return reinterpret_cast<T*>(reinterpret_cast<char*>(ws) + off);
}

static size_t head_smem_bytes(const rlx_ppo_dims& d, bool train) {
  size_t s = ((size_t)d.act_dim * d.hidden + d.hidden) * sizeof(float);
  if (train) s += (size_t)8 * (2 * d.act_dim + 5 + 2 * d.hidden) * sizeof(float);
  return s;
}

static int mlp_hidden_forward(const rlx_ppo_dims& d, const PpoLayout& L, const float* params, const float* X, long long ldx, long long rows,
                              float* H1, float* H2, cudaStream_t stream, int bf16 = 0) {
  const int H = L.H;
  const bool tc = use_tc(d);
  GemmP g{};
  g.A = X; g.B = params + L.off[W1P]; g.C = H1; g.bias = params + L.off[B1P];
  g.M = (int)rows; g.N = 2 * H; g.K = L.obs;
  g.lda = (int)ldx; g.ldb = L.obs; g.ldc = 2 * H;
  g.splits = 1; g.kchunk = (int)(ceil_div(L.obs, 8) * 8);
  g.bf16 = bf16;
  int rc = run_gemm<true, true, EPI_BIAS_TANH>(tc, g, 1, stream, KC_GEMM_FWD, rows, 2 * H);
  if (rc) return rc;
  GemmP g2{};
  g2.A = H1; g2.B = params + L.off[W2P]; g2.C = H2; g2.bias = params + L.off[B2P];
  g2.M = (int)rows; g2.N = H; g2.K = H;
  g2.lda = 2 * H; g2.ldb = H; g2.ldc = 2 * H;
  g2.sA = H; g2.sB = (long long)H * H; g2.sC = H; g2.sBias = H;
  g2.splits = 1; g2.kchunk = (int)(ceil_div(H, 8) * 8);
  g2.bf16 = bf16;
  return run_gemm<true, true, EPI_BIAS_TANH>(tc, g2, 2, stream, KC_GEMM_FWD, rows, H);
}

#define RLX_DISPATCH_NCH_1(CLS, FLOPS, BYTES, KERNEL, NCH_, BF_, grid, block, smem, stream, arg)                                    \
  do {                                                                                                                              \
    RLX_CHECK_CUDA(cudaFuncSetAttribute(KERNEL<NCH_, BF_>, cudaFuncAttributeMaxDynamicSharedMemorySize, (int)(smem)));              \
    RLX_LAUNCH_C(CLS, FLOPS, BYTES, (KERNEL<NCH_, BF_>), grid, block, smem, stream, arg);                                           \
  } while (0)
#define RLX_DISPATCH_NCH_B(CLS, FLOPS, BYTES, H, KERNEL, BF_, grid, block, smem, stream, arg)                                       \
  do {                                                                                                                              \
    const int _nch = (int)ceil_div((H), 32);                                                                                        \
    if (_nch <= 2) RLX_DISPATCH_NCH_1(CLS, FLOPS, BYTES, KERNEL, 2, BF_, grid, block, smem, stream, arg);                           \
    else if (_nch <= 4) RLX_DISPATCH_NCH_1(CLS, FLOPS, BYTES, KERNEL, 4, BF_, grid, block, smem, stream, arg);                      \
    else if (_nch <= 8) RLX_DISPATCH_NCH_1(CLS, FLOPS, BYTES, KERNEL, 8, BF_, grid, block, smem, stream, arg);                      \
    else if (_nch <= 16) RLX_DISPATCH_NCH_1(CLS, FLOPS, BYTES, KERNEL, 16, BF_, grid, block, smem, stream, arg);                    \
    else RLX_DISPATCH_NCH_1(CLS, FLOPS, BYTES, KERNEL, 32, BF_, grid, block, smem, stream, arg);                                    \
  } while (0)
#define RLX_DISPATCH_NCH(CLS, FLOPS, BYTES, H, KERNEL, grid, block, smem, stream, arg)                                              \
  do {                                                                                                                              \
    if ((arg).bf16) RLX_DISPATCH_NCH_B(CLS, FLOPS, BYTES, H, KERNEL, true, grid, block, smem, stream, arg);                         \
    else RLX_DISPATCH_NCH_B(CLS, FLOPS, BYTES, H, KERNEL, false, grid, block, smem, stream, arg);                                   \
  } while (0)

static bool head_dims_ok(const rlx_ppo_dims& d) {
  return dims_ok(d) && d.hidden <= 1024 && head_smem_bytes(d, true) <= 200 * 1024;
}

int ppo_head_gemm_path(const HeadGemmArgs& a, cudaStream_t st);
static int g_head_engine = 0;

static void fill_head_common(HeadP& h, const PpoLayout& L, const float* params, const float* H2, long long rows) {
  h.M = (int)rows; h.H = L.H; h.act = L.act;
  h.H2 = H2;
  h.W3p = params + L.off[W3P]; h.W3c = params + L.off[W3C];
  h.b3p = params + L.off[B3P]; h.b3c = params + L.off[B3C];
  h.logstd = params + L.off[LOGSTD];
}

}

using namespace rlx;

extern "C" size_t rlx_ppo_forward_workspace_bytes(const rlx_ppo_dims* d, int64_t n) {
  if (d == nullptr || !head_dims_ok(*d) || n < 0) return 0;
  return plan_forward(*d, n).total;
}

extern "C" int rlx_ppo_forward_f32(const rlx_ppo_forward_args* a, void* stream) {
  RLX_CHECK_ARG(a != nullptr, "args is null");
  RLX_CHECK_ARG(head_dims_ok(a->dims), "unsupported dims (act <= 64, hidden <= 1024)");
  RLX_CHECK_ARG(a->n >= 0 && a->n < (1LL << 31), "bad row count");
  if (a->n == 0) return RLX_OK;
  RLX_CHECK_ARG(a->params && a->obs, "params / obs is null");
  RLX_CHECK_ARG(!a->env_action || !a->clip_rescale || (a->act_low && a->act_high), "action bounds required for clip_rescale");
  const FwdPlan P = plan_forward(a->dims, a->n);
  if (a->workspace == nullptr || a->workspace_bytes < P.total) {
    set_error("rlx_ppo_forward_f32: workspace too small (%zu < %zu)", a->workspace_bytes, P.total);
    return RLX_ERR_WORKSPACE;
  }
  const PpoLayout L = make_layout(a->dims);
  float* H1 = ws_ptr<float>(a->workspace, P.off_H1);
  float* H2 = ws_ptr<float>(a->workspace, P.off_H2);
  cudaStream_t st = (cudaStream_t)stream;
  const int bf16 = g_autocast_bf16;
  const float* params = a->params;
  const float* obs = a->obs;
  int rc;
  if (bf16) {
    rc = round_inputs_bf16(L, params, obs, a->n * (long long)L.obs, ws_ptr<float>(a->workspace, P.off_P), ws_ptr<float>(a->workspace, P.off_X), st);
    if (rc) return rc;
  }
  rc = mlp_hidden_forward(a->dims, L, params, obs, a->dims.obs_dim, a->n, H1, H2, st, bf16);
  if (rc) return rc;
  HeadP h{};
  fill_head_common(h, L, params, H2, a->n);
  h.bf16 = bf16;
  h.noise = a->noise; h.seed = a->rng_seed; h.offset = a->rng_offset;
  h.act_low = a->act_low; h.act_high = a->act_high;
  h.clip_rescale = a->clip_rescale; h.deterministic = a->deterministic;
  h.action = a->action; h.env_action = a->env_action; h.logp_out = a->logp; h.value_out = a->value;
  const size_t smem = head_smem_bytes(a->dims, false);
  const int grid = head_grid(a->n);
  RLX_DISPATCH_NCH(KC_HEAD_ROLLOUT, 2.0 * a->n * L.H * (L.act + 1), 4.0 * a->n * (2.0 * L.H + 3.0 * L.act + 2), L.H, ppo_head_rollout_kernel, grid, 256, smem, st, h);
  return RLX_OK;
}

extern "C" int rlx_critic_forward_f32(const rlx_ppo_dims* d, const float* params, const float* obs, int64_t n, float* value,
                                      void* workspace, size_t workspace_bytes, void* stream) {
  RLX_CHECK_ARG(d != nullptr, "dims is null");
  rlx_ppo_forward_args a{};
  a.dims = *d; a.n = n; a.params = params; a.obs = obs; a.deterministic = 1; a.value = value;
  a.workspace = workspace; a.workspace_bytes = workspace_bytes;
  return rlx_ppo_forward_f32(&a, stream);
}

extern "C" size_t rlx_ppo_minibatch_workspace_bytes(const rlx_ppo_dims* d, int64_t m) {
  if (d == nullptr || !head_dims_ok(*d) || m < 0) return 0;
  return plan_train(*d, std::max<int64_t>(m, 1)).total;
}

static int check_mb_args(const rlx_ppo_minibatch_args* a, bool need_data, TrainPlan& P) {
  RLX_CHECK_ARG(a != nullptr, "args is null");
  RLX_CHECK_ARG(head_dims_ok(a->dims), "unsupported dims (act <= 64, hidden <= 1024)");
  RLX_CHECK_ARG(a->m >= 0 && a->m < (1LL << 31) && a->m_global >= 1, "bad minibatch size");
  RLX_CHECK_ARG(a->params && a->grads, "params / grads is null");
  if (need_data && a->m > 0) {
    RLX_CHECK_ARG(a->states && a->actions && a->log_probs && a->advantages && a->returns && a->adv_stats, "null minibatch tensor");
  }
  P = plan_train(a->dims, std::max<int64_t>(a->m, 1));
  if (a->workspace == nullptr || a->workspace_bytes < P.total) {
    set_error("rlx_ppo_minibatch: workspace too small (%zu < %zu)", a->workspace_bytes, P.total);
    return RLX_ERR_WORKSPACE;
  }
  return RLX_OK;
}

static long long tall_elements(const GradReduceP& r) {
  long long tall = 0;
  for (int gi = 0; gi < kNumGroups; ++gi)
    if (r.g[gi].nsplit > kTallSplit) tall += r.g[gi].len;
  return tall;
}
static double partial_bytes(const GradReduceP& r) {
  double b = 0;
  for (int gi = 0; gi < kNumGroups; ++gi) b += 4.0 * r.g[gi].nsplit * r.g[gi].len;
  return b;
}
static int launch_grad_reduce(const GradReduceP& r, cudaStream_t st) {
  const int flat_blocks = (int)ceil_div(r.total, 256);
  const int tall_blocks = (int)ceil_div(tall_elements(r), 8);
  RLX_LAUNCH_C(KC_GRAD_REDUCE, 0, partial_bytes(r) + 4.0 * r.total, ppo_grad_reduce_kernel, (unsigned)(flat_blocks + tall_blocks), 256, 0, st, r, flat_blocks);
  return RLX_OK;
}

static bool fast_head_ok(const PpoLayout& L) { return (L.act <= 31) && (L.H % 2 == 0) && (L.H <= 1024); }

static int launch_train_head(const rlx_ppo_minibatch_args* a, const PpoLayout& L, const TrainPlan& P, const float* params, int bf16, cudaStream_t st) {
  const long long m = a->m;
  const int H = L.H, A = L.act;
  void* ws = a->workspace;
  float* H2 = ws_ptr<float>(ws, P.off_H2);
  float* dZ2 = ws_ptr<float>(ws, P.off_dZ2);
  float* dhead = ws_ptr<float>(ws, P.off_dhead);
  float* headpart = ws_ptr<float>(ws, P.off_headpart);
  const float inv_mg = 1.f / (float)a->m_global;
  HeadP h{};
  fill_head_common(h, L, params, H2, m);
  h.bf16 = bf16;
  h.actions = a->actions; h.logp_old = a->log_probs; h.adv = a->advantages; h.ret = a->returns; h.adv_stats = a->adv_stats;
  h.inv_mg = inv_mg; h.clip_range = a->hp.clip_range; h.critic_coef = a->hp.critic_coef;
  h.ratio_delta_metric = a->hp.ratio_delta_metric != 0.f ? 1 : 0;
  const bool want_median = a->hp.ratio_delta_metric == 2.f;
  h.ratio_abs = want_median ? ws_ptr<float>(ws, P.off_ratio) : nullptr;
  h.dZ2 = dZ2; h.dhead = dhead; h.block_partials = headpart;
  int head_blocks = P.head_blocks;
  const size_t smem = head_smem_bytes(a->dims, true);
  const int dh_ld = (int)(ceil_div(A + 1, 4) * 4);
  const bool fast_head = fast_head_ok(L);
  const double head_flops = 4.0 * m * H * (A + 1), head_bytes = 4.0 * m * (4.0 * H + 2.0 * A + 5);
  const bool gemm_head = fast_head && g_head_engine == 1 && !bf16 && head_gemm_scratch_floats(m, H, A) <= m * 2LL * H;
  if (gemm_head) {
    HeadGemmArgs ha{m, H, A, dh_ld, H2, a->params + L.off[W3P], a->params + L.off[W3C], a->params + L.off[B3P], a->params + L.off[B3C],
                    a->params + L.off[LOGSTD], a->actions, a->log_probs, a->advantages, a->returns, a->adv_stats, inv_mg, a->hp.clip_range,
                    a->hp.critic_coef, a->hp.ratio_delta_metric != 0.f ? 1 : 0, dZ2, dhead, headpart, ws_ptr<float>(ws, P.off_dZ1)};
    const int rc = ppo_head_gemm_path(ha, st);
    if (rc) return rc;
    return 1;
  }
  if (!fast_head) {
    RLX_DISPATCH_NCH(KC_HEAD_TRAIN, head_flops, head_bytes, H, ppo_head_train_kernel, head_blocks, 256, smem, st, h);
    return head_blocks;
  }
  HeadTrain2Extra ex{dh_ld};
  const bool vec_head = (H == 128 || H == 256 || H == 512);
  const int nt4 = (int)ceil_div(dh_ld, 8);
  const size_t smem4 = head4_smem_floats(H, A, nt4) * sizeof(float);
  const bool mma_head = vec_head && g_head_engine == 2 && !bf16 && nt4 <= 4 && smem4 <= 220 * 1024;
  if (mma_head) {
    head_blocks = (int)std::min<long long>(ceil_div(m, 16 * kHead4RowTiles), (long long)P.head_blocks);
#define RLX_HEAD4(H_, NT_)                                                                                                          \
  do {                                                                                                                              \
    RLX_CHECK_CUDA(cudaFuncSetAttribute(ppo_head_train4_kernel<H_, NT_>, cudaFuncAttributeMaxDynamicSharedMemorySize, (int)smem4)); \
    RLX_LAUNCH_C(KC_HEAD_TRAIN, head_flops, head_bytes, (ppo_head_train4_kernel<H_, NT_>), head_blocks, 256, smem4, st, h, ex);     \
  } while (0)
#define RLX_HEAD4_NT(H_)              \
  do {                                \
    if (nt4 == 1) RLX_HEAD4(H_, 1);   \
    else if (nt4 == 2) RLX_HEAD4(H_, 2); \
    else if (nt4 == 3) RLX_HEAD4(H_, 3); \
    else RLX_HEAD4(H_, 4);            \
  } while (0)
    if (H == 128) RLX_HEAD4_NT(128);
    else if (H == 256) RLX_HEAD4_NT(256);
    else RLX_HEAD4_NT(512);
#undef RLX_HEAD4_NT
#undef RLX_HEAD4
  } else if (vec_head) {
#define RLX_HEAD3_B(H_, AM_, BF_)                                                                                                     \
  do {                                                                                                                                \
    RLX_CHECK_CUDA(cudaFuncSetAttribute(ppo_head_train3_kernel<H_, AM_, BF_>, cudaFuncAttributeMaxDynamicSharedMemorySize, (int)smem)); \
    RLX_LAUNCH_C(KC_HEAD_TRAIN, head_flops, head_bytes, (ppo_head_train3_kernel<H_, AM_, BF_>), head_blocks, 256, smem, st, h, ex);    \
  } while (0)
#define RLX_HEAD3(H_, AM_)                          \
  do {                                              \
    if (bf16) RLX_HEAD3_B(H_, AM_, true);           \
    else RLX_HEAD3_B(H_, AM_, false);               \
  } while (0)
#define RLX_HEAD3_ACT(H_)                      \
  do {                                         \
    if (A <= 8) RLX_HEAD3(H_, 8);              \
    else if (A <= 16) RLX_HEAD3(H_, 16);       \
    else if (A <= 24) RLX_HEAD3(H_, 24);       \
    else RLX_HEAD3(H_, 31);                    \
  } while (0)
    if (H == 128) RLX_HEAD3_ACT(128);
    else if (H == 256) RLX_HEAD3_ACT(256);
    else RLX_HEAD3_ACT(512);
#undef RLX_HEAD3_ACT
#undef RLX_HEAD3
#undef RLX_HEAD3_B
  } else {
    const int nch = (int)ceil_div(H, 32);
#define RLX_HEAD2_B(NCH_, AM_, BF_)                                                                                                   \
  do {                                                                                                                                \
    RLX_CHECK_CUDA(cudaFuncSetAttribute(ppo_head_train2_kernel<NCH_, AM_, BF_>, cudaFuncAttributeMaxDynamicSharedMemorySize, (int)smem)); \
    RLX_LAUNCH_C(KC_HEAD_TRAIN, head_flops, head_bytes, (ppo_head_train2_kernel<NCH_, AM_, BF_>), head_blocks, 256, smem, st, h, ex);  \
  } while (0)
#define RLX_HEAD2(NCH_, AM_)                        \
  do {                                              \
    if (bf16) RLX_HEAD2_B(NCH_, AM_, true);         \
    else RLX_HEAD2_B(NCH_, AM_, false);             \
  } while (0)
#define RLX_HEAD2_ACT(NCH_)                         \
  do {                                              \
    if (A <= 8) RLX_HEAD2(NCH_, 8);                 \
    else if (A <= 16) RLX_HEAD2(NCH_, 16);          \
    else if (A <= 24) RLX_HEAD2(NCH_, 24);          \
    else RLX_HEAD2(NCH_, 31);                       \
  } while (0)
    if (nch <= 2) RLX_HEAD2_ACT(2);
    else if (nch <= 4) RLX_HEAD2_ACT(4);
    else if (nch <= 8) RLX_HEAD2_ACT(8);
    else if (nch <= 16) RLX_HEAD2_ACT(16);
    else RLX_HEAD2_ACT(32);
#undef RLX_HEAD2_ACT
#undef RLX_HEAD2
#undef RLX_HEAD2_B
  }
  return head_blocks;
}

struct W3Partials {
  float* src;
  int nsplit;
  long long stride, critic_off;
};
static W3Partials chunked_w3(const PpoLayout& L, float* part3, int nchunks) {
  return W3Partials{part3, nchunks, (long long)(L.act + 1) * L.H, (long long)L.act * L.H};
}

static int launch_head_wgrad(const PpoLayout& L, const TrainPlan& P, long long m, bool tc, int bf16, void* ws, cudaStream_t st, W3Partials& w3) {
  const int H = L.H, A = L.act;
  float* H2 = ws_ptr<float>(ws, P.off_H2);
  float* dhead = ws_ptr<float>(ws, P.off_dhead);
  float* part3 = ws_ptr<float>(ws, P.off_part3);
  const int wgrad_chunks = (int)ceil_div(m, kHeadWgradRows);
  const double wflops = 2.0 * m * H * (A + 1), wbytes = 4.0 * m * (2.0 * H + A + 1);
  if (!fast_head_ok(L)) {
    HeadWgradP w{(int)m, H, A, kHeadWgradRows, H2, dhead, part3};
    dim3 wg((unsigned)wgrad_chunks, (unsigned)ceil_div(2 * H, 256));
    const size_t wsmem = (size_t)kHeadWgradRows * (A + 1) * sizeof(float);
    if (A <= 8) RLX_LAUNCH_C(KC_HEAD_WGRAD, wflops, wbytes, ppo_head_wgrad_kernel<8>, wg, 256, wsmem, st, w);
    else if (A <= 32) RLX_LAUNCH_C(KC_HEAD_WGRAD, wflops, wbytes, ppo_head_wgrad_kernel<32>, wg, 256, wsmem, st, w);
    else {
      RLX_CHECK_CUDA(cudaFuncSetAttribute(ppo_head_wgrad_kernel<64>, cudaFuncAttributeMaxDynamicSharedMemorySize, (int)wsmem));
      RLX_LAUNCH_C(KC_HEAD_WGRAD, wflops, wbytes, ppo_head_wgrad_kernel<64>, wg, 256, wsmem, st, w);
    }
    w3 = chunked_w3(L, part3, wgrad_chunks);
    return RLX_OK;
  }
  const int dh_ld = (int)(ceil_div(A + 1, 4) * 4);
  if (tc) {
    const Splits S3 = choose_splits(m, dh_ld, H, 2, true);
    GemmP g3{};
    g3.A = dhead; g3.B = H2; g3.C = part3;
    g3.M = dh_ld; g3.N = H; g3.K = (int)m;
    g3.lda = dh_ld; g3.ldb = 2 * H; g3.ldc = H;
    g3.sA = 0; g3.sB = H; g3.sC = (long long)dh_ld * H;
    g3.splits = S3.splits; g3.kchunk = S3.kchunk; g3.sSplitC = 2LL * dh_ld * H;
    g3.bf16 = bf16;
    const int rc = tc_gemm(g3, false, false, TC_NONE, 2, KC_HEAD_WGRAD, m, m, st);
    if (rc == RLX_OK) {
      w3 = W3Partials{part3, S3.splits, 2LL * dh_ld * H, (long long)dh_ld * H + (long long)A * H};
      return RLX_OK;
    }
    if (rc != RLX_ERR_UNSUPPORTED) return rc;
  }
  HeadWgrad2P w{(int)m, H, A, dh_ld, kHeadWgradRows, H2, dhead, part3};
  const unsigned wthreads = (unsigned)(ceil_div(H, 32) * 32);
  const size_t wsmem = (size_t)kHeadWgradRows * dh_ld * sizeof(float);
  if (A + 1 <= 4) RLX_LAUNCH_C(KC_HEAD_WGRAD, wflops, wbytes, ppo_head_wgrad3_kernel<4>, wgrad_chunks, wthreads, wsmem, st, w);
  else if (A + 1 <= 8) RLX_LAUNCH_C(KC_HEAD_WGRAD, wflops, wbytes, ppo_head_wgrad3_kernel<8>, wgrad_chunks, wthreads, wsmem, st, w);
  else if (A + 1 <= 12) RLX_LAUNCH_C(KC_HEAD_WGRAD, wflops, wbytes, ppo_head_wgrad3_kernel<12>, wgrad_chunks, wthreads, wsmem, st, w);
  else if (A + 1 <= 16) RLX_LAUNCH_C(KC_HEAD_WGRAD, wflops, wbytes, ppo_head_wgrad3_kernel<16>, wgrad_chunks, wthreads, wsmem, st, w);
  else if (A + 1 <= 20) RLX_LAUNCH_C(KC_HEAD_WGRAD, wflops, wbytes, ppo_head_wgrad3_kernel<20>, wgrad_chunks, wthreads, wsmem, st, w);
  else if (A + 1 <= 24) RLX_LAUNCH_C(KC_HEAD_WGRAD, wflops, wbytes, ppo_head_wgrad3_kernel<24>, wgrad_chunks, wthreads, wsmem, st, w);
  else RLX_LAUNCH_C(KC_HEAD_WGRAD, wflops, wbytes, ppo_head_wgrad3_kernel<32>, wgrad_chunks, wthreads, wsmem, st, w);
  w3 = chunked_w3(L, part3, wgrad_chunks);
  return RLX_OK;
}

static int launch_hidden_backward(const PpoLayout& L, const TrainPlan& P, const float* params, const float* states, long long ldx, bool ones_col,
                                  long long m, bool tc, int bf16, void* ws, cudaStream_t st, int& s1, int& s2) {
  const int H = L.H, O = L.obs;
  float* H1 = ws_ptr<float>(ws, P.off_H1);
  float* dZ2 = ws_ptr<float>(ws, P.off_dZ2);
  float* dZ1 = ws_ptr<float>(ws, P.off_dZ1);
  float* part1 = ws_ptr<float>(ws, P.off_part1);
  float* rs1 = ws_ptr<float>(ws, P.off_rs1);
  float* part2 = ws_ptr<float>(ws, P.off_part2);
  const Splits S2 = choose_splits(m, H, H, 2, tc);
  s2 = S2.splits;
  GemmP g{};
  g.A = dZ2; g.B = H1; g.C = part2;
  g.M = H; g.N = H; g.K = (int)m;
  g.lda = 2 * H; g.ldb = 2 * H; g.ldc = H;
  g.sA = H; g.sB = H; g.sC = (long long)H * H;
  g.splits = S2.splits; g.kchunk = S2.kchunk; g.sSplitC = 2LL * H * H;
  g.bf16 = bf16;
  int rc = run_gemm<false, false, EPI_NONE>(tc, g, 2, st, KC_GEMM_DW, m, m);
  if (rc) return rc;
  GemmP gd{};
  gd.A = dZ2; gd.B = params + L.off[W2P]; gd.C = dZ1; gd.aux = H1;
  gd.bf16 = bf16;
  gd.M = (int)m; gd.N = H; gd.K = H;
  gd.lda = 2 * H; gd.ldb = H; gd.ldc = 2 * H; gd.ldaux = 2 * H;
  gd.sA = H; gd.sB = (long long)H * H; gd.sC = H; gd.sAux = H;
  gd.splits = 1; gd.kchunk = (int)(ceil_div(H, 8) * 8);
  rc = run_gemm<true, false, EPI_DTANH>(tc, gd, 2, st, KC_GEMM_DX, m, H);
  if (rc) return rc;
  if (tc && ones_col) {
    const Splits S1 = choose_splits(m, O + 1, 2 * H, 1, true);
    GemmP gt{};
    gt.A = states; gt.B = dZ1; gt.C = part1;
    gt.bf16 = bf16;
    gt.M = O + 1; gt.N = 2 * H; gt.K = (int)m;
    gt.lda = (int)ldx; gt.ldb = 2 * H; gt.ldc = O;
    gt.splits = S1.splits; gt.kchunk = S1.kchunk; gt.sSplitC = 2LL * H * O;
    rc = tc_gemm_t(gt, false, false, TC_NONE, 1, KC_GEMM_DW, m, m, O, rs1, 0, 2LL * H, st);
    if (rc == RLX_OK) {
      s1 = S1.splits;
      return RLX_OK;
    }
    if (rc != RLX_ERR_UNSUPPORTED) return rc;
  }
  const Splits S1 = choose_splits(m, 2 * H, O, 1, false);
  s1 = S1.splits;
  GemmP g1{};
  g1.A = dZ1; g1.B = states; g1.C = part1;
  g1.bf16 = bf16;
  g1.M = 2 * H; g1.N = O; g1.K = (int)m;
  g1.lda = 2 * H; g1.ldb = (int)ldx; g1.ldc = O;
  g1.rowsum = rs1;
  g1.splits = S1.splits; g1.kchunk = S1.kchunk; g1.sSplitC = 2LL * H * O; g1.sSplitRowsum = 2LL * H;
  return launch_sgemm<false, false, EPI_NONE>(g1, 1, st, KC_GEMM_DW);
}

static GradReduceP make_grad_reduce(const rlx_ppo_minibatch_args* a, const PpoLayout& L, const TrainPlan& P, int head_blocks, const W3Partials& w3,
                                    int s1, int s2, bool fuse_norms) {
  const int H = L.H, O = L.obs, A = L.act;
  void* ws = a->workspace;
  const float* headpart = ws_ptr<float>(ws, P.off_headpart);
  const int npart = P.head_npart;
  const float inv_mg = 1.f / (float)a->m_global;
  GradReduceP r{};
  r.g[0] = GradGroup{L.off[W1P], 2LL * H * O, ws_ptr<float>(ws, P.off_part1), s1, 2LL * H * O};
  r.g[1] = GradGroup{L.off[B1P], 2LL * H, ws_ptr<float>(ws, P.off_rs1), s1, 2LL * H};
  r.g[2] = GradGroup{L.off[W2P], 2LL * H * H, ws_ptr<float>(ws, P.off_part2), s2, 2LL * H * H};
  r.g[3] = GradGroup{L.off[B2P], 2LL * H, headpart + (2 * A + 5), head_blocks, (long long)npart};
  r.g[4] = GradGroup{L.off[W3P], (long long)A * H, w3.src, w3.nsplit, w3.stride};
  r.g[5] = GradGroup{L.off[B3P], 2LL * A + 1, headpart, head_blocks, (long long)npart};
  r.g[6] = GradGroup{L.off[W3C], (long long)H, w3.src + w3.critic_off, w3.nsplit, w3.stride};
  r.total = L.total();
  r.logstd_off = L.off[LOGSTD];
  r.act = A;
  r.entropy_grad = -a->hp.entropy_coef * (float)a->m * inv_mg;
  r.grads = a->grads;
  r.head_partials = headpart; r.nblk = head_blocks; r.npart = npart; r.inv_mg = inv_mg; r.critic_coef = a->hp.critic_coef;
  r.logstd = a->params + L.off[LOGSTD];
  r.metrics = a->metrics; r.m_local = (float)a->m;
  r.bf16 = g_autocast_bf16;
  if (fuse_norms) {
    r.norm_partials = ws_ptr<float>(ws, P.off_norm);
    r.done = ws_ptr<unsigned int>(ws, P.off_barrier);
    r.norm_out = ws_ptr<float>(ws, P.off_barrier) + 4;
    r.step_count = (long long*)a->step_count;
    r.net = make_net_map(L);
  }
  return r;
}

static int minibatch_fwdbwd(const rlx_ppo_minibatch_args* a, void* stream, bool fuse_norms = false) {
  TrainPlan P;
  int rc = check_mb_args(a, true, P);
  if (rc) return rc;
  const PpoLayout L = make_layout(a->dims);
  const long long m = a->m;
  const long long ldx = a->states_ld > 0 ? a->states_ld : L.obs;
  RLX_CHECK_ARG(ldx >= L.obs, "states_ld smaller than obs_dim");
  RLX_CHECK_ARG(!a->states_ones_col || ldx > L.obs, "states_ones_col needs states_ld > obs_dim");
  const bool tc = use_tc(a->dims);
  const int bf16 = g_autocast_bf16;
  cudaStream_t st = (cudaStream_t)stream;
  void* ws = a->workspace;
  int head_blocks = 0, s1 = 0, s2 = 0;
  W3Partials w3 = chunked_w3(L, ws_ptr<float>(ws, P.off_part3), 0);
  if (m > 0) {
    const float* params = a->params;
    const float* states = a->states;
    if (bf16) {
      RLX_CHECK_ARG(ldx <= (long long)(ceil_div(L.obs + 1, 4) * 4), "bf16 mode: states_ld larger than the planned rounded copy");
      rc = round_inputs_bf16(L, params, states, m * ldx, ws_ptr<float>(ws, P.off_P), ws_ptr<float>(ws, P.off_X), st);
      if (rc) return rc;
    }
    rc = mlp_hidden_forward(a->dims, L, params, states, ldx, m, ws_ptr<float>(ws, P.off_H1), ws_ptr<float>(ws, P.off_H2), st, bf16);
    if (rc) return rc;
    head_blocks = launch_train_head(a, L, P, params, bf16, st);
    if (head_blocks < 0) return head_blocks;
    rc = launch_head_wgrad(L, P, m, tc, bf16, ws, st, w3);
    if (rc) return rc;
    rc = launch_hidden_backward(L, P, params, states, ldx, a->states_ones_col, m, tc, bf16, ws, st, s1, s2);
    if (rc) return rc;
  }
  rc = launch_grad_reduce(make_grad_reduce(a, L, P, head_blocks, w3, s1, s2, fuse_norms), st);
  if (rc) return rc;
  if (a->hp.ratio_delta_metric == 2.f && m > 0 && a->metrics != nullptr) {
    RLX_LAUNCH_C(KC_OTHER, 0, 16.0 * m, median_lower_kernel, 1, 1024, 0, st, ws_ptr<float>(ws, P.off_ratio), (long long)m, a->metrics + 4);
  }
  return RLX_OK;
}

extern "C" int rlx_ppo_minibatch_fwdbwd_f32(const rlx_ppo_minibatch_args* a, void* stream) { return minibatch_fwdbwd(a, stream); }

static AdamP make_adam_params(const rlx_ppo_minibatch_args* a, const PpoLayout& L, float* norm_partials, int nblk_norm) {
  AdamP p{};
  p.total = L.total();
  p.net = make_net_map(L);
  p.params = a->params; p.grads = a->grads; p.m = a->exp_avg; p.v = a->exp_avg_sq;
  p.lr = a->lr; p.step_count = (long long*)a->step_count;
  p.max_norm = a->hp.max_grad_norm; p.beta1 = a->hp.adam_beta1; p.beta2 = a->hp.adam_beta2; p.eps = a->hp.adam_eps;
  p.norm_partials = norm_partials;
  p.nblk_norm = nblk_norm;
  p.metrics = a->metrics;
  return p;
}

static int launch_clip_adam(const rlx_ppo_minibatch_args* a, const PpoLayout& L, float* norm_partials, int nblk, cudaStream_t st) {
  const AdamP p = make_adam_params(a, L, norm_partials, nblk);
  RLX_LAUNCH_C(KC_CLIP_ADAM, 0, 28.0 * L.total(), ppo_clip_adam_kernel, (unsigned)ceil_div(L.total(), 256), 256, 0, st, p);
  return RLX_OK;
}

extern "C" int rlx_gradnorm_clip_adam_f32(const rlx_ppo_minibatch_args* a, void* stream) {
  TrainPlan P;
  int rc = check_mb_args(a, false, P);
  if (rc) return rc;
  RLX_CHECK_ARG(a->exp_avg && a->exp_avg_sq && a->lr && a->step_count, "optimizer state is null");
  const PpoLayout L = make_layout(a->dims);
  cudaStream_t st = (cudaStream_t)stream;
  const int nblk = 64;
  float* partials = ws_ptr<float>(a->workspace, P.off_norm);
  const AdamP p = make_adam_params(a, L, partials, nblk);
  RLX_LAUNCH_C(KC_CLIP_ADAM, 0, 4.0 * L.total(), ppo_grad_sumsq_kernel, (unsigned)nblk, 256, 0, st, p);
  return launch_clip_adam(a, L, partials, nblk, st);
}

static rlx_ppo_minibatch_args minibatch_slice(const rlx_ppo_minibatch_args* first, int64_t k, int64_t r0, int64_t m) {
  const int64_t ld = first->states_ld > 0 ? first->states_ld : first->dims.obs_dim;
  rlx_ppo_minibatch_args a = *first;
  a.m = m;
  a.states = first->states + r0 * ld;
  a.actions = first->actions + r0 * first->dims.act_dim;
  a.log_probs = first->log_probs + r0;
  a.advantages = first->advantages + r0;
  a.returns = first->returns + r0;
  a.adv_stats = first->adv_stats + 2 * k;
  return a;
}

extern "C" int rlx_ppo_update_epoch_f32(const rlx_ppo_minibatch_args* first, int64_t count, int64_t mb, void* stream) {
  RLX_CHECK_ARG(first != nullptr && count >= 0 && mb > 0, "bad arguments");
  const int64_t nmb = ceil_div(count, mb), full = std::min<int64_t>(mb, count);
  cudaStream_t st = (cudaStream_t)stream;
  bool norms_in_reduce = dims_ok(first->dims) && first->exp_avg && first->exp_avg_sq && first->lr && first->step_count && first->workspace;
  TrainPlan P{};
  if (norms_in_reduce) {
    P = plan_train(first->dims, std::max<int64_t>(full, 1));
    if (first->workspace_bytes < P.total) norms_in_reduce = false;
    else RLX_CHECK_CUDA(cudaMemsetAsync(ws_ptr<unsigned int>(first->workspace, P.off_barrier), 0, 64, st));
  }
  for (int64_t k = 0; k < nmb; ++k) {
    rlx_ppo_minibatch_args a = minibatch_slice(first, k, k * mb, std::min<int64_t>(mb, count - k * mb));
    a.m_global = a.m;
    a.metrics = first->metrics ? first->metrics + RLX_PPO_NMETRIC * k : nullptr;
    int rc;
    if (norms_in_reduce && a.m == full) {
      rc = minibatch_fwdbwd(&a, stream, true);
      if (rc) return rc;
      rc = launch_clip_adam(&a, make_layout(a.dims), ws_ptr<float>(a.workspace, P.off_barrier) + 4, 1, st);
    } else {
      rc = minibatch_fwdbwd(&a, stream);
      if (rc) return rc;
      rc = rlx_gradnorm_clip_adam_f32(&a, stream);
    }
    if (rc) return rc;
  }
  return RLX_OK;
}

extern "C" int rlx_ppo_update_epoch_sharded_f32(const rlx_ppo_minibatch_args* first, int64_t num_mb, const int64_t* counts,
                                                const int64_t* global_counts, rlx_comm* comm, void* stream) {
  RLX_CHECK_ARG(first != nullptr && num_mb >= 0 && counts && global_counts && comm, "bad arguments");
  RLX_CHECK_ARG(first->metrics != nullptr, "metrics rows are required");
  const PpoLayout L = make_layout(first->dims);
  const int64_t P = L.total();
  cudaStream_t st = (cudaStream_t)stream;
  int64_t r0 = 0;
  for (int64_t k = 0; k < num_mb; ++k) {
    RLX_CHECK_ARG(counts[k] >= 0 && global_counts[k] >= 1, "bad minibatch sizes");
    rlx_ppo_minibatch_args a = minibatch_slice(first, k, r0, counts[k]);
    a.m_global = global_counts[k];
    float* send = rlx_comm_send_buffer(comm);
    a.grads = send;
    a.metrics = send + P;
    int rc = minibatch_fwdbwd(&a, stream);
    if (rc) return rc;
    float* norm_partials = ws_ptr<float>(a.workspace, plan_train(a.dims, std::max<int64_t>(a.m, 1)).off_norm);
    int nblk = 0;
    rc = comm_allreduce_ppo(comm, first->grads, P + RLX_PPO_NMETRIC, a.dims, norm_partials, (long long*)a.step_count, stream, &nblk);
    if (rc) return rc;
    a.grads = first->grads;
    a.metrics = first->grads + P;
    if (nblk > 0) {
      RLX_CHECK_ARG(a.exp_avg && a.exp_avg_sq && a.lr && a.step_count, "optimizer state is null");
      rc = launch_clip_adam(&a, L, norm_partials, nblk, st);
    } else {
      rc = rlx_gradnorm_clip_adam_f32(&a, stream);
    }
    if (rc) return rc;
    RLX_CHECK_CUDA(cudaMemcpyAsync(first->metrics + RLX_PPO_NMETRIC * k, first->grads + P, RLX_PPO_NMETRIC * sizeof(float),
                                   cudaMemcpyDeviceToDevice, st));
    r0 += counts[k];
  }
  return RLX_OK;
}

extern "C" int rlx_debug_gemm_f32(int engine, int layout, int epilogue, int64_t M, int64_t N, int64_t K, const float* A, int64_t lda,
                                  const float* B, int64_t ldb, float* C, int64_t ldc, const float* bias, const float* aux, int64_t ldaux,
                                  void* stream) {
  RLX_CHECK_ARG(A && B && C && M > 0 && N > 0 && K > 0, "bad arguments");
  RLX_CHECK_ARG(engine == 0 || engine == 1, "unknown engine (0 = SIMT, 1 = wgmma tensor cores)");
  const bool bias_epi = epilogue == 1 || epilogue == 3 || epilogue == 5, aux_epi = epilogue == 2 || epilogue == 4;
  RLX_CHECK_ARG((epilogue == 0) || (bias_epi && layout == 0 && bias) || (aux_epi && layout == 1 && aux) ||
                    (epilogue == 6 && layout == 2 && engine == 1 && M >= 2),
                "unsupported epilogue/layout");
  GemmP g{};
  g.A = A; g.B = B; g.C = C; g.bias = bias; g.aux = aux;
  g.M = (int)M; g.N = (int)N; g.K = (int)K;
  g.lda = (int)lda; g.ldb = (int)ldb; g.ldc = (int)ldc; g.ldaux = (int)ldaux;
  g.splits = 1; g.kchunk = (int)(ceil_div(K, 8) * 8);
  cudaStream_t st = (cudaStream_t)stream;
  const bool a_k = layout != 2, b_k = layout == 0;
  const long long a_rows = a_k ? M : K, b_rows = b_k ? N : K;
  if (engine == 1) {
    const int rc = epilogue == 6 ? tc_gemm_t(g, a_k, b_k, TC_NONE, 1, KC_OTHER, a_rows, b_rows, (int)M - 1, C + N * ldc, 0, 0, st)
                                 : tc_gemm(g, a_k, b_k, epilogue, 1, KC_OTHER, a_rows, b_rows, st);
    if (rc == RLX_ERR_UNSUPPORTED) set_error("rlx_debug_gemm_f32: shape/alignment not supported by the wgmma engine");
    return rc;
  }
  if (layout == 0 && epilogue == 1) return launch_sgemm<true, true, EPI_BIAS_TANH>(g, 1, st);
  if (layout == 0 && epilogue == 3) return launch_sgemm<true, true, EPI_BIAS_RELU>(g, 1, st);
  if (layout == 0 && epilogue == 5) return launch_sgemm<true, true, EPI_BIAS>(g, 1, st);
  if (layout == 0) return launch_sgemm<true, true, EPI_NONE>(g, 1, st);
  if (layout == 1 && epilogue == 2) return launch_sgemm<true, false, EPI_DTANH>(g, 1, st);
  if (layout == 1 && epilogue == 4) return launch_sgemm<true, false, EPI_DRELU>(g, 1, st);
  if (layout == 1) return launch_sgemm<true, false, EPI_NONE>(g, 1, st);
  return launch_sgemm<false, false, EPI_NONE>(g, 1, st);
}

extern "C" int rlx_set_head_engine(int engine) {
  if (engine >= 0 && engine <= 2) g_head_engine = engine;
  else set_error("rlx_set_head_engine: unknown engine %d", engine);
  return g_head_engine;
}

extern "C" int rlx_set_gemm_engine(int engine) {
  if (engine != 0 && engine != 1) {
    set_error("rlx_set_gemm_engine: unknown engine %d", engine);
    return g_gemm_engine;
  }
  g_gemm_engine = engine;
  return g_gemm_engine;
}
```

Measured before the change: 3.027 million.

## Pre-split weights into TF32 hi/lo once per minibatch for tensor-core GEMMs

Adds a kernel that splits the weight matrices (W1, W2 and a transposed W2) into TF32 high and low parts once per minibatch and stores them in workspace. The wgmma GEMM kernel gains a SPLIT_B variant that TMA-loads both parts straight into shared memory, so consumers no longer convert raw B tiles to hi/lo operands inside every tile. This removes the per-tile conversion stage and its separate operand buffers and barriers. The cost is an extra split launch, doubled B-operand memory traffic and extra workspace.

```diff
diff --git a/include/rlx_b200.h b/include/rlx_b200.h
--- a/include/rlx_b200.h
+++ b/include/rlx_b200.h
@@ -31,6 +31,7 @@
 int rlx_debug_gemm_f32(int engine, int layout, int epilogue, int64_t M, int64_t N, int64_t K, const float* A, int64_t lda,
                        const float* B, int64_t ldb, float* C, int64_t ldc, const float* bias, const float* aux, int64_t ldaux,
                        void* stream);
+int rlx_debug_tf32_split_f32(const float* src, int64_t batch, int64_t rows, int64_t cols, int trans, float* hi, float* lo, void* stream);
 
 typedef struct rlx_pcg64 { uint64_t s[6]; } rlx_pcg64;
 int rlx_pcg64_seed(uint64_t seed, rlx_pcg64* st);
diff --git a/rl_x_b200/_native.py b/rl_x_b200/_native.py
--- a/rl_x_b200/_native.py
+++ b/rl_x_b200/_native.py
@@ -228,6 +228,7 @@
     "rlx_gather_minibatch_f32": (C.c_int, [C.c_void_p, C.c_int64, C.c_int64, C.c_int64] + [C.c_void_p] * 10 + [C.c_int64, C.c_void_p]),
     "rlx_debug_gemm_f32": (C.c_int, [C.c_int, C.c_int, C.c_int, C.c_int64, C.c_int64, C.c_int64, C.c_void_p, C.c_int64, C.c_void_p, C.c_int64,
                                      C.c_void_p, C.c_int64, C.c_void_p, C.c_void_p, C.c_int64, C.c_void_p]),
+    "rlx_debug_tf32_split_f32": (C.c_int, [C.c_void_p, C.c_int64, C.c_int64, C.c_int64, C.c_int, C.c_void_p, C.c_void_p, C.c_void_p]),
     "rlx_advantage_stats_f32": (C.c_int, [C.c_void_p, C.c_int64, C.c_int64, C.c_void_p, C.c_void_p]),
     "rlx_segment_moments_f32": (C.c_int, [C.c_void_p, C.c_void_p, C.c_int64, C.c_void_p, C.c_void_p, C.c_void_p, C.c_void_p]),
     "rlx_ppo_minibatch_workspace_bytes": (C.c_size_t, [C.POINTER(PpoDims), C.c_int64]),
diff --git a/rl_x_b200/algorithms/ppo/b200/kernels.py b/rl_x_b200/algorithms/ppo/b200/kernels.py
--- a/rl_x_b200/algorithms/ppo/b200/kernels.py
+++ b/rl_x_b200/algorithms/ppo/b200/kernels.py
@@ -132,6 +132,12 @@
         nt.check(self.lib.rlx_debug_gemm_f32(int(engine), int(layout), int(epilogue), M, N, K, _f32(A, "A"), A.stride(0), _f32(B, "B"), B.stride(0),
                                              _f32(C, "C"), C.stride(0), _f32(bias, "bias"), _f32(aux, "aux"), aux.stride(0) if aux is not None else 0,
                                              _stream()), "rlx_debug_gemm_f32")
+
+    def debug_tf32_split(self, src, trans, hi, lo):
+        assert src.dim() == 3 and src.is_contiguous() and hi.is_contiguous() and lo.is_contiguous()
+        b, r, c = src.shape
+        nt.check(self.lib.rlx_debug_tf32_split_f32(_f32(src, "src"), b, r, c, int(bool(trans)), _f32(hi, "hi"), _f32(lo, "lo"), _stream()),
+                 "rlx_debug_tf32_split_f32")
 
     def states_pitch(self):
         return (self.obs_dim + 1 + 3) // 4 * 4
diff --git a/rl_x_b200/csrc/gemm_dispatch.cuh b/rl_x_b200/csrc/gemm_dispatch.cuh
--- a/rl_x_b200/csrc/gemm_dispatch.cuh
+++ b/rl_x_b200/csrc/gemm_dispatch.cuh
@@ -8,6 +8,15 @@
 int tc_gemm_t(const GemmP& g, bool a_kmaj, bool b_kmaj, int epi, int batch, int kclass, long long a_rows, long long b_rows, int m_main, float* extra_row,
               long long extra_batch_off, long long extra_split_off, cudaStream_t stream);
 enum { TC_NONE = 0, TC_BIAS_TANH = 1, TC_DTANH = 2, TC_BIAS_RELU = 3, TC_DRELU = 4, TC_BIAS = 5 };
+
+struct Tf32SplitJob {
+  const float* src;
+  float* hi;
+  float* lo;
+  int batch, rows, cols, trans;
+};
+constexpr int kMaxTf32SplitJobs = 3;
+int tf32_split(const Tf32SplitJob* jobs, int njobs, int kclass, cudaStream_t stream);
 
 template <int EPI>
 constexpr int tc_epi_of() {
diff --git a/rl_x_b200/csrc/gemm_simt.cuh b/rl_x_b200/csrc/gemm_simt.cuh
--- a/rl_x_b200/csrc/gemm_simt.cuh
+++ b/rl_x_b200/csrc/gemm_simt.cuh
@@ -19,6 +19,8 @@
   int kchunk;
   long long sSplitC, sSplitRowsum;
   int bf16;
+  const float* b_hi;
+  const float* b_lo;
 };
 
 constexpr int GBM = 128, GBN = 128, GBK = 8, GPAD = 4;
diff --git a/rl_x_b200/csrc/gemm_tc.cu b/rl_x_b200/csrc/gemm_tc.cu
--- a/rl_x_b200/csrc/gemm_tc.cu
+++ b/rl_x_b200/csrc/gemm_tc.cu
@@ -11,9 +11,12 @@
   static constexpr int OP_BYTES = 2 * B_BYTES;
   static constexpr int RAW_STAGES = 3, OP_STAGES = 4;
   static constexpr int SMEM_BYTES = RAW_STAGES * RAW_BYTES + OP_STAGES * OP_BYTES + 1024  + 1024 ;
+  static constexpr int SPLIT_STAGE_BYTES = A_BYTES + 2 * B_BYTES;
+  static constexpr int SPLIT_STAGES = 4;
+  static constexpr int SPLIT_SMEM_BYTES = SPLIT_STAGES * SPLIT_STAGE_BYTES + 1024 + 1024;
   static constexpr int PRODUCER_REGS = 56, CONSUMER_REGS = 224;
 };
-static_assert(Cfg::SMEM_BYTES <= 227 * 1024, "shared memory of one H100 block");
+static_assert(Cfg::SMEM_BYTES <= 227 * 1024 && Cfg::SPLIT_SMEM_BYTES <= 227 * 1024, "shared memory of one H100 block");
 static_assert(Cfg::PRODUCER_REGS * 128 + Cfg::CONSUMER_REGS * 256 <= 65536, "register file of one SM");
 
 template <bool KMAJ, bool BF16, int ROWS>
@@ -154,14 +157,16 @@
   }
 }
 
-template <bool A_KMAJ, bool B_KMAJ, int EPI, bool BF16, bool TRANS>
-__global__ void __launch_bounds__(NUM_THREADS, 1) tc_gemm_kernel(const __grid_constant__ CUtensorMap tmap_a,
-                                                                 const __grid_constant__ CUtensorMap tmap_b, const TcParams p) {
-  constexpr int RAW_STAGES = Cfg::RAW_STAGES, OP_STAGES = Cfg::OP_STAGES;
+template <bool A_KMAJ, bool B_KMAJ, int EPI, bool BF16, bool TRANS, bool SPLIT_B>
+__global__ void __launch_bounds__(NUM_THREADS, 1) tc_gemm_kernel(const __grid_constant__ CUtensorMap tmap_a, const __grid_constant__ CUtensorMap tmap_b,
+                                                                 const __grid_constant__ CUtensorMap tmap_b_lo, const TcParams p) {
+  static_assert(!SPLIT_B || (B_KMAJ && !BF16), "pre-split B is K-major fp32 hi / lo");
+  constexpr int RAW_STAGES = SPLIT_B ? Cfg::SPLIT_STAGES : Cfg::RAW_STAGES, OP_STAGES = SPLIT_B ? Cfg::SPLIT_STAGES : Cfg::OP_STAGES;
+  constexpr int RAW_BYTES = SPLIT_B ? Cfg::SPLIT_STAGE_BYTES : Cfg::RAW_BYTES;
   extern __shared__ uint8_t smem_raw[];
   uint8_t* smem = smem_raw + ((1024u - (smem_u32(smem_raw) & 1023u)) & 1023u);
-  uint8_t* ops = smem + RAW_STAGES * Cfg::RAW_BYTES;
-  uint64_t* raw_full = reinterpret_cast<uint64_t*>(ops + OP_STAGES * Cfg::OP_BYTES);
+  uint8_t* ops = smem + RAW_STAGES * RAW_BYTES;
+  uint64_t* raw_full = reinterpret_cast<uint64_t*>(ops + (SPLIT_B ? 0 : OP_STAGES * Cfg::OP_BYTES));
   uint64_t* raw_empty = raw_full + RAW_STAGES;
   uint64_t* op_full = raw_empty + RAW_STAGES;
   uint64_t* op_empty = op_full + OP_STAGES;
@@ -170,6 +175,7 @@
   if (threadIdx.x == 0) {
     prefetch_tmap(&tmap_a);
     prefetch_tmap(&tmap_b);
+    if (SPLIT_B) prefetch_tmap(&tmap_b_lo);
     for (int s = 0; s < RAW_STAGES; ++s) {
       mbar_init(&raw_full[s], 1);
       mbar_init(&raw_empty[s], 1 + 8);
@@ -199,6 +205,7 @@
   if (warp < 4) {
     setmaxnreg_dec<Cfg::PRODUCER_REGS>();
     const int t = threadIdx.x;
+    uint64_t* ld_empty = SPLIT_B ? op_empty : raw_empty;
     int ld_tile = blockIdx.x, ld_kb = 0, ld_count = 0;
     auto load_next = [&]() {
       while (ld_tile < num_tiles) {
@@ -210,12 +217,12 @@
           continue;
         }
         const int slot = ld_count % RAW_STAGES;
-        mbar_wait(&raw_empty[slot], ((ld_count / RAW_STAGES) & 1) ^ 1);
-        uint8_t* sa = smem + slot * Cfg::RAW_BYTES;
+        mbar_wait(&ld_empty[slot], ((ld_count / RAW_STAGES) & 1) ^ 1);
+        uint8_t* sa = smem + slot * RAW_BYTES;
         uint8_t* sb = sa + Cfg::A_BYTES;
         uint64_t* bar = &raw_full[slot];
         const int k0 = kbeg + ld_kb * BK;
-        mbar_arrive_expect_tx(bar, Cfg::RAW_BYTES);
+        mbar_arrive_expect_tx(bar, RAW_BYTES);
         if (A_KMAJ) {
           tma_load_2d(&tmap_a, bar, sa, p.a_k_off * zb + k0, p.a_mn_off * zb + m0);
         } else {
@@ -224,15 +231,23 @@
         }
         if (B_KMAJ) {
           tma_load_2d(&tmap_b, bar, sb, p.b_k_off * zb + k0, p.b_mn_off * zb + n0);
+          if (SPLIT_B) tma_load_2d(&tmap_b_lo, bar, sb + Cfg::B_BYTES, p.b_k_off * zb + k0, p.b_mn_off * zb + n0);
         } else {
 #pragma unroll
           for (int j = 0; j < BN / 32; ++j) tma_load_2d(&tmap_b, bar, sb + j * (BK * 128), p.b_mn_off * zb + n0 + 32 * j, p.b_k_off * zb + k0);
         }
         ++ld_kb;
         ++ld_count;
-        return;
-      }
+        return true;
+      }
+      return false;
     };
+    if constexpr (SPLIT_B) {
+      if (t == 0)
+        while (load_next()) {
+        }
+      return;
+    }
     if (t == 0)
       for (int i = 0; i < RAW_STAGES; ++i) load_next();
     int rs = 0, os = 0;
@@ -271,14 +286,14 @@
       tile_coords(tile, zb, zs, m0, n0, kbeg, nkb);
       for (int kb = 0; kb < nkb; ++kb) {
         mbar_wait(&raw_full[rs], rph);
-        mbar_wait(&op_full[os], oph);
-        const uint8_t* raw = smem + rs * Cfg::RAW_BYTES;
-        const uint32_t op = smem_u32(ops + os * Cfg::OP_BYTES);
+        if (!SPLIT_B) mbar_wait(&op_full[os], oph);
+        const uint8_t* raw = smem + rs * RAW_BYTES;
+        const uint32_t op = SPLIT_B ? smem_u32(raw + Cfg::A_BYTES) : smem_u32(ops + os * Cfg::OP_BYTES);
         const uint64_t db = make_smem_desc(op), db_lo = make_smem_desc(op + Cfg::B_BYTES);
 #pragma unroll
         for (int h = 0; h < 2; ++h) {
           load_a_frags<A_KMAJ, BF16>(raw, r0, lane, h, ah[h], al[h]);
-          if (h == 1) {
+          if (!SPLIT_B && h == 1) {
             __syncwarp();
             if (lane == 0) mbar_arrive(&raw_empty[rs]);
           }
@@ -339,28 +354,35 @@
   }
 }
 
-template <bool A_KMAJ, bool B_KMAJ, int EPI, bool BF16 = false, bool TRANS = false>
-static int launch_cfg(const TcOperand& A, const TcOperand& B, TcParams p, int kclass, cudaStream_t stream) {
-  CUtensorMap ta, tb;
+template <bool A_KMAJ, bool B_KMAJ, int EPI, bool BF16 = false, bool TRANS = false, bool SPLIT_B = false>
+static int launch_cfg(const TcOperand& A, const TcOperand& B, TcParams p, int kclass, cudaStream_t stream, const float* b_lo = nullptr) {
+  CUtensorMap ta, tb, tb_lo;
   int rc = make_tmap(&ta, A.base, A.rows, A.cols, A.ld, 32, A_KMAJ ? BM : BK);
   if (rc) return rc;
   rc = make_tmap(&tb, B.base, B.rows, B.cols, B.ld, 32, B_KMAJ ? BN : BK);
   if (rc) return rc;
+  if (SPLIT_B) {
+    rc = make_tmap(&tb_lo, b_lo, B.rows, B.cols, B.ld, 32, BN);
+    if (rc) return rc;
+  } else {
+    tb_lo = tb;
+  }
   p.tiles_m = (int)ceil_div(p.M, BM);
   p.tiles_n = (int)ceil_div(p.N, BN);
   const long long tiles = (long long)p.tiles_m * p.tiles_n * p.batch * p.splits;
   if (tiles <= 0) return RLX_OK;
   static_assert(!TRANS || EPI == TC_EPI_NONE, "the transposed store has no epilogue function");
-  auto kern = tc_gemm_kernel<A_KMAJ, B_KMAJ, EPI, BF16, TRANS>;
+  auto kern = tc_gemm_kernel<A_KMAJ, B_KMAJ, EPI, BF16, TRANS, SPLIT_B>;
+  constexpr int smem = SPLIT_B ? Cfg::SPLIT_SMEM_BYTES : Cfg::SMEM_BYTES;
   static bool attr_done = false;
   if (!attr_done) {
-    RLX_CHECK_CUDA(cudaFuncSetAttribute(kern, cudaFuncAttributeMaxDynamicSharedMemorySize, Cfg::SMEM_BYTES));
+    RLX_CHECK_CUDA(cudaFuncSetAttribute(kern, cudaFuncAttributeMaxDynamicSharedMemorySize, smem));
     attr_done = true;
   }
   const unsigned grid = (unsigned)std::min<long long>(tiles, sm_count());
   const double flops = 2.0 * p.M * p.N * (double)p.K * p.batch;
-  const double bytes = 4.0 * p.batch * ((double)p.M * p.K + (double)p.N * p.K + (double)p.M * p.N * p.splits);
-  RLX_LAUNCH_C(kclass, flops, bytes, kern, grid, NUM_THREADS, Cfg::SMEM_BYTES, stream, ta, tb, p);
+  const double bytes = 4.0 * p.batch * ((double)p.M * p.K + (SPLIT_B ? 2.0 : 1.0) * p.N * p.K + (double)p.M * p.N * p.splits);
+  RLX_LAUNCH_C(kclass, flops, bytes, kern, grid, NUM_THREADS, smem, stream, ta, tb, tb_lo, p);
   return RLX_OK;
 }
 
@@ -377,6 +399,12 @@
 static int tc_gemm_impl(const GemmP& g, bool a_kmaj, bool b_kmaj, int epi, int batch, int kclass, long long a_rows, long long b_rows, bool trans,
                         int m_main, float* extra_row, long long extra_batch_off, long long extra_split_off, cudaStream_t stream) {
   if (g.M <= 0 || g.N <= 0) return RLX_OK;
+  const bool split_b = g.b_hi != nullptr && !g.bf16 && !trans && a_kmaj && (epi == TC_EPI_BIAS_TANH || epi == TC_EPI_DTANH);
+  if (split_b) {
+    if (!aligned16(g.b_hi) || !aligned16(g.b_lo)) return RLX_ERR_UNSUPPORTED;
+    b_kmaj = true;
+    b_rows = g.N;
+  }
   if (!aligned16(g.A) || !aligned16(g.B) || !aligned16(g.C) || g.lda % 4 || g.ldb % 4 || g.ldc % 4) return RLX_ERR_UNSUPPORTED;
   if (g.splits > 1 && g.kchunk % BK) return RLX_ERR_UNSUPPORTED;
   if (!trans && (((batch > 1 ? g.sC : 0) | (g.splits > 1 ? g.sSplitC : 0)) & 1)) return RLX_ERR_UNSUPPORTED;
@@ -387,6 +415,7 @@
       for (int b = 0; b < batch; ++b) {
         GemmP gb = g;
         gb.A = g.A + b * g.sA; gb.B = g.B + b * g.sB; gb.C = g.C + b * g.sC;
+        if (g.b_hi) { gb.b_hi = g.b_hi + b * g.sB; gb.b_lo = g.b_lo + b * g.sB; }
         if (g.bias) gb.bias = g.bias + b * g.sBias;
         if (g.aux) gb.aux = g.aux + b * g.sAux;
         gb.sA = gb.sB = gb.sC = gb.sBias = gb.sAux = 0;
@@ -417,7 +446,7 @@
   p.bf16 = g.bf16;
   TcOperand A{g.A, (a_kmaj ? (long long)p.a_mn_off : (long long)p.a_k_off) * (batch - 1) + a_rows,
               a_kmaj ? (long long)(p.a_k_off * (batch - 1) + g.K) : (long long)(p.a_mn_off * (batch - 1) + g.M), g.lda};
-  TcOperand B{g.B, (b_kmaj ? (long long)p.b_mn_off : (long long)p.b_k_off) * (batch - 1) + b_rows,
+  TcOperand B{split_b ? g.b_hi : g.B, (b_kmaj ? (long long)p.b_mn_off : (long long)p.b_k_off) * (batch - 1) + b_rows,
               b_kmaj ? (long long)(p.b_k_off * (batch - 1) + g.K) : (long long)(p.b_mn_off * (batch - 1) + g.N), g.ldb};
   if (trans) {
     if (!a_kmaj && !b_kmaj && epi == TC_EPI_NONE)
@@ -429,6 +458,8 @@
   if (p.bf16 && a_kmaj && !b_kmaj && epi == TC_EPI_DTANH) return launch_cfg<true, false, TC_EPI_DTANH, true>(A, B, p, kclass, stream);
   if (p.bf16 && !a_kmaj && !b_kmaj && epi == TC_EPI_NONE) return launch_cfg<false, false, TC_EPI_NONE, true>(A, B, p, kclass, stream);
   if (p.bf16) return RLX_ERR_UNSUPPORTED;
+  if (split_b && epi == TC_EPI_BIAS_TANH) return launch_cfg<true, true, TC_EPI_BIAS_TANH, false, false, true>(A, B, p, kclass, stream, g.b_lo);
+  if (split_b && epi == TC_EPI_DTANH) return launch_cfg<true, true, TC_EPI_DTANH, false, false, true>(A, B, p, kclass, stream, g.b_lo);
   if (a_kmaj && b_kmaj && epi == TC_EPI_BIAS_TANH) return launch_cfg<true, true, TC_EPI_BIAS_TANH>(A, B, p, kclass, stream);
   if (a_kmaj && b_kmaj && epi == TC_EPI_NONE) return launch_cfg<true, true, TC_EPI_NONE>(A, B, p, kclass, stream);
   if (a_kmaj && b_kmaj && epi == TC_EPI_BIAS_RELU) return launch_cfg<true, true, TC_EPI_BIAS_RELU>(A, B, p, kclass, stream);
@@ -449,4 +480,54 @@
   return tc_gemm_impl(g, a_kmaj, b_kmaj, epi, batch, kclass, a_rows, b_rows, true, m_main, extra_row, extra_batch_off, extra_split_off, stream);
 }
 
-}
+namespace tc {
+struct Tf32SplitJobs {
+  Tf32SplitJob job[kMaxTf32SplitJobs];
+  int first_tile[kMaxTf32SplitJobs + 1];
+};
+
+__global__ void __launch_bounds__(256) tf32_split_kernel(const __grid_constant__ Tf32SplitJobs J) {
+  __shared__ float tile[32][33];
+  int j = 0;
+  while ((int)blockIdx.x >= J.first_tile[j + 1]) ++j;
+  const Tf32SplitJob& s = J.job[j];
+  const int tiles_c = (s.cols + 31) / 32, tiles_rc = ((s.rows + 31) / 32) * tiles_c;
+  const int b = (int)blockIdx.x - J.first_tile[j];
+  const int z = b / tiles_rc, r0 = (b % tiles_rc) / tiles_c * 32, c0 = b % tiles_c * 32;
+  const long long zoff = (long long)z * s.rows * s.cols;
+  const int tx = threadIdx.x & 31, ty = threadIdx.x >> 5;
+#pragma unroll
+  for (int i = ty; i < 32; i += 8)
+    if (r0 + i < s.rows && c0 + tx < s.cols) tile[i][tx] = s.src[zoff + (long long)(r0 + i) * s.cols + c0 + tx];
+  __syncthreads();
+#pragma unroll
+  for (int i = ty; i < 32; i += 8) {
+    const int dr = s.trans ? c0 + i : r0 + i, dc = s.trans ? r0 + tx : c0 + tx, dcols = s.trans ? s.rows : s.cols;
+    if (dr < (s.trans ? s.cols : s.rows) && dc < dcols) {
+      const float x = s.trans ? tile[tx][i] : tile[i][tx];
+      const uint32_t h = __float_as_uint(x) & 0xFFFFE000u;
+      const long long o = zoff + (long long)dr * dcols + dc;
+      s.hi[o] = __uint_as_float(h);
+      s.lo[o] = x - __uint_as_float(h);
+    }
+  }
+}
+}
+
+int tf32_split(const Tf32SplitJob* jobs, int njobs, int kclass, cudaStream_t stream) {
+  if (njobs < 1 || njobs > kMaxTf32SplitJobs) return RLX_ERR_INVALID_ARG;
+  Tf32SplitJobs J{};
+  long long tiles = 0, elems = 0;
+  for (int i = 0; i < njobs; ++i) {
+    J.job[i] = jobs[i];
+    J.first_tile[i] = (int)tiles;
+    tiles += (long long)jobs[i].batch * ceil_div(jobs[i].rows, 32) * ceil_div(jobs[i].cols, 32);
+    elems += (long long)jobs[i].batch * jobs[i].rows * jobs[i].cols;
+  }
+  for (int i = njobs; i <= kMaxTf32SplitJobs; ++i) J.first_tile[i] = (int)tiles;
+  if (tiles == 0) return RLX_OK;
+  RLX_LAUNCH_C(kclass, 0, 12.0 * elems, tf32_split_kernel, (unsigned)tiles, 256, 0, stream, J);
+  return RLX_OK;
+}
+
+}
diff --git a/rl_x_b200/csrc/ppo.cu b/rl_x_b200/csrc/ppo.cu
--- a/rl_x_b200/csrc/ppo.cu
+++ b/rl_x_b200/csrc/ppo.cu
@@ -80,8 +80,11 @@
 
 constexpr int kHeadWgradRows = 64;
 
+enum { WS_W1_HI, WS_W1_LO, WS_W2_HI, WS_W2_LO, WS_W2T_HI, WS_W2T_LO, WS_COUNT };
+
 struct TrainPlan {
   size_t off_H1, off_H2, off_dZ2, off_dZ1, off_dhead, off_headpart, off_part1, off_rs1, off_part2, off_part3, off_norm, off_barrier, off_P, off_X, off_ratio, total;
+  size_t off_wsplit[WS_COUNT];
   int max_s1, max_s2, max_s3;
   int head_blocks, wgrad_chunks, norm_blocks, head_npart;
 };
@@ -118,6 +121,7 @@
   take(P.off_P, (size_t)make_layout(d).total());
   take(P.off_X, (size_t)m * (size_t)(ceil_div(O + 1, 4) * 4));
   take(P.off_ratio, (size_t)m);
+  for (int i = 0; i < WS_COUNT; ++i) take(P.off_wsplit[i], i < WS_W2_HI ? (size_t)(2 * H * O) : (size_t)(2 * H * H));
   P.total = o;
   return P;
 }
@@ -133,8 +137,21 @@
   return s;
 }
 
+struct SplitWeights {
+  const float* p[WS_COUNT];
+};
+static int split_weights(const PpoLayout& L, const float* params, void* ws, const TrainPlan& P, SplitWeights& sw, cudaStream_t st) {
+  const int H = L.H;
+  float* w[WS_COUNT];
+  for (int i = 0; i < WS_COUNT; ++i) sw.p[i] = w[i] = ws_ptr<float>(ws, P.off_wsplit[i]);
+  const Tf32SplitJob jobs[3] = {{params + L.off[W1P], w[WS_W1_HI], w[WS_W1_LO], 1, 2 * H, L.obs, 0},
+                                {params + L.off[W2P], w[WS_W2_HI], w[WS_W2_LO], 1, 2 * H, H, 0},
+                                {params + L.off[W2P], w[WS_W2T_HI], w[WS_W2T_LO], 2, H, H, 1}};
+  return tf32_split(jobs, 3, KC_GEMM_FWD, st);
+}
+
 static int mlp_hidden_forward(const rlx_ppo_dims& d, const PpoLayout& L, const float* params, const float* X, long long ldx, long long rows,
-                              float* H1, float* H2, cudaStream_t stream, int bf16 = 0) {
+                              float* H1, float* H2, cudaStream_t stream, int bf16 = 0, const SplitWeights* sw = nullptr) {
   const int H = L.H;
   const bool tc = use_tc(d);
   GemmP g{};
@@ -143,10 +160,12 @@
   g.lda = (int)ldx; g.ldb = L.obs; g.ldc = 2 * H;
   g.splits = 1; g.kchunk = (int)(ceil_div(L.obs, 8) * 8);
   g.bf16 = bf16;
+  if (sw) { g.b_hi = sw->p[WS_W1_HI]; g.b_lo = sw->p[WS_W1_LO]; }
   int rc = run_gemm<true, true, EPI_BIAS_TANH>(tc, g, 1, stream, KC_GEMM_FWD, rows, 2 * H);
   if (rc) return rc;
   GemmP g2{};
   g2.A = H1; g2.B = params + L.off[W2P]; g2.C = H2; g2.bias = params + L.off[B2P];
+  if (sw) { g2.b_hi = sw->p[WS_W2_HI]; g2.b_lo = sw->p[WS_W2_LO]; }
   g2.M = (int)rows; g2.N = H; g2.K = H;
   g2.lda = 2 * H; g2.ldb = H; g2.ldc = 2 * H;
   g2.sA = H; g2.sB = (long long)H * H; g2.sC = H; g2.sBias = H;
@@ -464,7 +483,7 @@
 }
 
 static int launch_hidden_backward(const PpoLayout& L, const TrainPlan& P, const float* params, const float* states, long long ldx, bool ones_col,
-                                  long long m, bool tc, int bf16, void* ws, cudaStream_t st, int& s1, int& s2) {
+                                  long long m, bool tc, int bf16, const SplitWeights* sw, void* ws, cudaStream_t st, int& s1, int& s2) {
   const int H = L.H, O = L.obs;
   float* H1 = ws_ptr<float>(ws, P.off_H1);
   float* dZ2 = ws_ptr<float>(ws, P.off_dZ2);
@@ -490,6 +509,7 @@
   gd.lda = 2 * H; gd.ldb = H; gd.ldc = 2 * H; gd.ldaux = 2 * H;
   gd.sA = H; gd.sB = (long long)H * H; gd.sC = H; gd.sAux = H;
   gd.splits = 1; gd.kchunk = (int)(ceil_div(H, 8) * 8);
+  if (sw) { gd.b_hi = sw->p[WS_W2T_HI]; gd.b_lo = sw->p[WS_W2T_LO]; }
   rc = run_gemm<true, false, EPI_DTANH>(tc, gd, 2, st, KC_GEMM_DX, m, H);
   if (rc) return rc;
   if (tc && ones_col) {
@@ -576,13 +596,20 @@
       rc = round_inputs_bf16(L, params, states, m * ldx, ws_ptr<float>(ws, P.off_P), ws_ptr<float>(ws, P.off_X), st);
       if (rc) return rc;
     }
-    rc = mlp_hidden_forward(a->dims, L, params, states, ldx, m, ws_ptr<float>(ws, P.off_H1), ws_ptr<float>(ws, P.off_H2), st, bf16);
+    SplitWeights sw{};
+    const bool presplit = tc && !bf16;
+    if (presplit) {
+      rc = split_weights(L, params, ws, P, sw, st);
+      if (rc) return rc;
+    }
+    rc = mlp_hidden_forward(a->dims, L, params, states, ldx, m, ws_ptr<float>(ws, P.off_H1), ws_ptr<float>(ws, P.off_H2), st, bf16,
+                            presplit ? &sw : nullptr);
     if (rc) return rc;
     head_blocks = launch_train_head(a, L, P, params, bf16, st);
     if (head_blocks < 0) return head_blocks;
     rc = launch_head_wgrad(L, P, m, tc, bf16, ws, st, w3);
     if (rc) return rc;
-    rc = launch_hidden_backward(L, P, params, states, ldx, a->states_ones_col, m, tc, bf16, ws, st, s1, s2);
+    rc = launch_hidden_backward(L, P, params, states, ldx, a->states_ones_col, m, tc, bf16, presplit ? &sw : nullptr, ws, st, s1, s2);
     if (rc) return rc;
   }
   rc = launch_grad_reduce(make_grad_reduce(a, L, P, head_blocks, w3, s1, s2, fuse_norms), st);
@@ -714,8 +741,10 @@
   RLX_CHECK_ARG(A && B && C && M > 0 && N > 0 && K > 0, "bad arguments");
   RLX_CHECK_ARG(engine == 0 || engine == 1, "unknown engine (0 = SIMT, 1 = wgmma tensor cores)");
   const bool bias_epi = epilogue == 1 || epilogue == 3 || epilogue == 5, aux_epi = epilogue == 2 || epilogue == 4;
-  RLX_CHECK_ARG((epilogue == 0) || (bias_epi && layout == 0 && bias) || (aux_epi && layout == 1 && aux) ||
-                    (epilogue == 6 && layout == 2 && engine == 1 && M >= 2),
+  const bool presplit = layout == 3 || layout == 4;
+  RLX_CHECK_ARG((epilogue == 0 && !presplit) || (bias_epi && layout == 0 && bias) || (aux_epi && layout == 1 && aux) ||
+                    (epilogue == 6 && layout == 2 && engine == 1 && M >= 2) ||
+                    (engine == 1 && layout == 3 && epilogue == 1 && bias) || (engine == 1 && layout == 4 && epilogue == 2 && aux && K % 4 == 0),
                 "unsupported epilogue/layout");
   GemmP g{};
   g.A = A; g.B = B; g.C = C; g.bias = bias; g.aux = aux;
@@ -723,6 +752,20 @@
   g.lda = (int)lda; g.ldb = (int)ldb; g.ldc = (int)ldc; g.ldaux = (int)ldaux;
   g.splits = 1; g.kchunk = (int)(ceil_div(K, 8) * 8);
   cudaStream_t st = (cudaStream_t)stream;
+  if (presplit) {
+    const int rows = (int)(layout == 3 ? N : K);
+    float* hi = nullptr;
+    RLX_CHECK_CUDA(cudaMallocAsync(reinterpret_cast<void**>(&hi), 2 * sizeof(float) * rows * ldb, st));
+    const Tf32SplitJob job{B, hi, hi + rows * ldb, 1, rows, (int)ldb, layout == 4};
+    int rc = tf32_split(&job, 1, KC_OTHER, st);
+    if (rc == RLX_OK) {
+      g.b_hi = job.hi; g.b_lo = job.lo;
+      if (layout == 4) g.ldb = (int)K;
+      rc = tc_gemm(g, true, layout == 3, epilogue, 1, KC_OTHER, M, layout == 3 ? N : K, st);
+    }
+    RLX_CHECK_CUDA(cudaFreeAsync(hi, st));
+    return rc;
+  }
   const bool a_k = layout != 2, b_k = layout == 0;
   const long long a_rows = a_k ? M : K, b_rows = b_k ? N : K;
   if (engine == 1) {
@@ -741,6 +784,12 @@
   return launch_sgemm<false, false, EPI_NONE>(g, 1, st);
 }
 
+extern "C" int rlx_debug_tf32_split_f32(const float* src, int64_t batch, int64_t rows, int64_t cols, int trans, float* hi, float* lo, void* stream) {
+  RLX_CHECK_ARG(src && hi && lo && batch > 0 && rows > 0 && cols > 0 && batch * rows * cols < (1LL << 31), "bad arguments");
+  const Tf32SplitJob job{src, hi, lo, (int)batch, (int)rows, (int)cols, trans ? 1 : 0};
+  return tf32_split(&job, 1, KC_OTHER, (cudaStream_t)stream);
+}
+
 extern "C" int rlx_set_head_engine(int engine) {
   if (engine >= 0 && engine <= 2) g_head_engine = engine;
   else set_error("rlx_set_head_engine: unknown engine %d", engine);
```

New measurement: 3.308 million, median of 6. 1.09x the previous value.
